# yumingj/C2-Matching

Hardware: AMD Instinct MI355X
Metric: LR-Ref image pairs/sec (160x160 LR, 500x500 Ref, 4x SR) (higher is better)
Workload: dtype f32

## Files before the change

c2-matching_amd/c2m_amd/_lib.py:

```python
import ctypes
import os

import torch

_HERE = os.path.dirname(os.path.abspath(__file__))
LIB_PATH = os.environ.get("C2M_LIB") or os.path.join(os.path.dirname(_HERE), "csrc", "libc2m_hip.so")
ABI_VERSION = 5

_vp, _i, _sz = ctypes.c_void_p, ctypes.c_int, ctypes.c_size_t
_lib = None


class ConvSrc(ctypes.Structure):
    _fields_ = [("ptr", _vp), ("C", _i), ("pix_pitch", _i), ("row_pitch", _i), ("img_pitch", ctypes.c_longlong)]


class Conv3x3Desc(ctypes.Structure):
    _fields_ = [("B", _i), ("H", _i), ("W", _i), ("Cin", _i), ("Cout", _i), ("nsrc", _i), ("src", ConvSrc * 2),
                ("wr", _vp), ("bias", _vp), ("act", _i), ("slope", ctypes.c_float), ("out_mode", _i), ("out", _vp),
                ("out_pix_pitch", _i), ("out_row_pitch", _i), ("out_img_pitch", ctypes.c_longlong), ("res1", _vp),
                ("res2", _vp), ("mask_out", _vp), ("flow", _vp), ("fh", _i), ("fw", _i), ("scale", _i), ("n_off", _i),
                ("abs_sum", _vp), ("algo", _i), ("cout_offset", _i), ("cout_total", _i),
                ("out2", _vp), ("out2_row_pitch", _i), ("out2_plane_pitch", ctypes.c_longlong),
                ("out2_img_pitch", ctypes.c_longlong), ("range_flag", _vp), ("io_flags", ctypes.c_int)]


class ImageSrc(ctypes.Structure):
    _fields_ = [("ptr", _vp), ("pix_pitch", ctypes.c_longlong), ("row_pitch", ctypes.c_longlong),
                ("plane_pitch", ctypes.c_longlong), ("img_pitch", ctypes.c_longlong)]


class C2MError(RuntimeError):
    pass


def _declare(L):
    L.c2m_abi_version.restype = _i
    L.c2m_status_string.restype = ctypes.c_char_p
    L.c2m_status_string.argtypes = [_i]
    L.c2m_last_hip_error.restype = ctypes.c_char_p
    L.c2m_device_arch.argtypes = [ctypes.c_char_p, _i]
    L.c2m_profile_enable.argtypes = [_i]
    L.c2m_profile_collect.argtypes = [ctypes.POINTER(ctypes.c_float), ctypes.POINTER(_i), _i, ctypes.POINTER(_i)]
    L.c2m_feature_normalize_f32.argtypes = [_vp, _vp, _i, _i, _i, _vp]
    L.c2m_feature_match_workspace_bytes.restype = _sz
    L.c2m_feature_match_workspace_bytes.argtypes = [_i] * 5
    L.c2m_feature_match_workspace_bytes_c.restype = _sz
    L.c2m_feature_match_workspace_bytes_c.argtypes = [_i] * 6
    L.c2m_feature_match_skip_table.argtypes = [_i] * 5 + [ctypes.POINTER(ctypes.c_size_t), ctypes.POINTER(ctypes.c_int)]
    L.c2m_feature_match_index_f32.argtypes = [_vp, _vp, _vp] + [_i] * 12 + [_vp, _vp, _vp, _sz]
    L.c2m_feature_match_index_pre_f32.argtypes = [_vp, _vp, _vp] + [_i] * 12 + [_vp, _vp, _vp, _sz, _vp, _vp]
    L.c2m_feature_match_index_pre_f32.restype = _i
    L.c2m_feature_normalize_ss_f32.argtypes = [_vp, _vp, _i, _i, _i, _vp, _vp]
    L.c2m_feature_normalize_ss_f32.restype = _i
    L.c2m_feature_match_filter_tables.argtypes = [_i] * 5 + [ctypes.POINTER(ctypes.c_size_t)] * 3 + [ctypes.POINTER(ctypes.c_int)]
    L.c2m_build_pre_offsets_f32.argtypes = [_vp, _vp, _i, _i, _i, _vp, _vp, _vp]
    for name in ("c2m_dcn_v2_forward_workspace_bytes",):
        getattr(L, name).restype = _sz
        getattr(L, name).argtypes = [_i] * 8
    L.c2m_dcn_v2_backward_workspace_bytes.restype = _sz
    L.c2m_dcn_v2_backward_workspace_bytes.argtypes = [_i] * 14
    L.c2m_dcn_v2_forward_f32.argtypes = [_vp] * 6 + [_i] * 14 + [_vp, _vp, _sz]
    L.c2m_dcn_v2_forward_bf16mma_f32.argtypes = [_vp] * 6 + [_i] * 14 + [_vp, _vp, _sz]
    L.c2m_dcn_v2_backward_f32.argtypes = [_vp] * 7 + [_i] * 14 + [_vp] * 5 + [_vp, _sz]
    L.c2m_dcn_fuse_offsets_f32.argtypes = [_vp, _vp, _vp, _i, _i, _i, _i, _i, _vp, _vp, _vp]
    L.c2m_nchw_to_nhwc_bordered_f32.argtypes = [_vp, _vp, _i, _i, _i, _i, _vp]
    L.c2m_dcn_v2_relayout_bytes.restype = _sz
    L.c2m_dcn_v2_relayout_bytes.argtypes = [_i] * 5
    L.c2m_dcn_v2_relayout_f32.argtypes = [_vp, _vp, _i, _i, _i, _i, _i, _vp]
    L.c2m_conv3x3_rgb64_f32.argtypes = [_vp, _vp, _i, _i, _i, _vp, _vp, _vp, _vp, _i, ctypes.c_float, _vp, _i, _i,
                                        ctypes.c_longlong, _vp, _i, ctypes.c_longlong, ctypes.c_longlong]
    L.c2m_dcn_v2_forward_nhwc_f32.argtypes = [_vp] * 6 + [_i] * 14 + [_vp, _i, _i, _i, ctypes.c_longlong, _i, ctypes.c_float, _i]
    L.c2m_dcn_v2_relayout_f16x2_bytes.restype = _sz
    L.c2m_dcn_v2_relayout_f16x2_bytes.argtypes = [_i] * 5
    L.c2m_dcn_v2_relayout_f16x2.argtypes = [_vp, _vp, _i, _i, _i, _i, _i, _vp]
    L.c2m_dcn_v2_forward_nhwc_f16x2.argtypes = [_vp] * 6 + [_i] * 14 + [_vp, _i, _i, _i, ctypes.c_longlong, _i, ctypes.c_float, _i, _vp]
    L.c2m_conv3x3_relayout_bytes.restype = _sz
    L.c2m_conv3x3_relayout_bytes.argtypes = [_i, _i]
    L.c2m_conv3x3_relayout_f32.argtypes = [_vp, _vp, _i, _i, _vp]
    L.c2m_conv3x3_relayout_wino_bytes.restype = _sz
    L.c2m_conv3x3_relayout_wino_bytes.argtypes = [_i, _i]
    L.c2m_conv3x3_relayout_wino_f32.argtypes = [_vp, _vp, _i, _i, _vp]
    L.c2m_conv3x3_relayout_wino4_bytes.restype = _sz
    L.c2m_conv3x3_relayout_wino4_bytes.argtypes = [_i, _i]
    L.c2m_conv3x3_relayout_wino4_f32.argtypes = [_vp, _vp, _i, _i, _vp]
    L.c2m_conv3x3_relayout_split_bytes.restype = _sz
    L.c2m_conv3x3_relayout_split_bytes.argtypes = [_i, _i, _i]
    L.c2m_conv3x3_relayout_split_f32.argtypes = [_vp, _vp, _i, _i, _i, _vp]
    L.c2m_conv3x3_relayout_split_dgrad_f32.argtypes = [_vp, _vp, _i, _i, _i, _vp]
    L.c2m_conv3x3_relayout_split_multi.argtypes = [_vp, _vp, _i, ctypes.c_longlong, _i]
    L.c2m_conv3x3_wgrad_workspace_bytes.restype = _sz
    L.c2m_conv3x3_wgrad_workspace_bytes.argtypes = [_i] * 5
    L.c2m_conv3x3_wgrad_f32.argtypes = [_vp, ctypes.POINTER(ConvSrc), _i, _vp, _i, _i, ctypes.c_longlong] + [_i] * 5 + [_vp, _vp, _sz]
    L.c2m_conv3x3_nhwc_f32.argtypes = [_vp, ctypes.POINTER(Conv3x3Desc)]
    L.c2m_index_to_flow_f32.argtypes = [_vp, _vp, _i, _i, _i, _vp]
    L.c2m_contras_loss_workspace_bytes.restype = _sz
    L.c2m_contras_loss_workspace_bytes.argtypes = [_i] * 6
    L.c2m_contras_loss_forward_f32.argtypes = [_vp] * 5 + [_i] * 6 + [_vp] * 3 + [_i, _i] + [ctypes.c_float] * 3 + [_vp, _vp, _sz]
    L.c2m_contras_loss_rows_f32.argtypes = [_vp] + [_i] * 6 + [_vp, _sz] + [_vp] * 5
    L.c2m_contras_loss_backward_f32.argtypes = [_vp] + [_i] * 6 + [_vp] * 3 + [_i, _i] + [ctypes.c_float] * 3 + [_i] + [_vp] * 4 + [_sz]
    L.c2m_warp_perspective_u8.argtypes = [_vp] * 4 + [_i] * 3 + [_vp] * 3
    L.c2m_pil_bicubic_u8.argtypes = [_vp, _vp] + [_i] * 5 + [_vp] * 3 + [_i, _vp, _vp]
    L.c2m_pil_bicubic2d_lds_bytes.restype = _sz
    L.c2m_pil_bicubic2d_lds_bytes.argtypes = [_i] * 4
    L.c2m_pil_bicubic2d_u8.argtypes = [_vp] * 3 + [_i] * 6 + ([_vp] * 3 + [_i]) * 2 + [_i, _i] + [_vp] * 3
    L.c2m_val_metrics_tile.argtypes = [ctypes.POINTER(_i)] * 2
    L.c2m_val_metrics_workspace_bytes.restype = _sz
    L.c2m_val_metrics_workspace_bytes.argtypes = [_i] * 4
    L.c2m_val_metrics_f32.argtypes = [_vp, ctypes.POINTER(ImageSrc), ctypes.POINTER(ImageSrc)] + [_i] * 7 + [_vp] * 4 + [_sz]


def lib():
    global _lib
    if _lib is None:
        if not os.path.exists(LIB_PATH):
            raise C2MError(f"{LIB_PATH} not found: build it with `python -c 'import __graft_entry__ as g; g.build()'` "
                           "(hipcc --offload-arch=gfx950).  There is no CPU or PyTorch fallback for this path.")
        L = ctypes.CDLL(LIB_PATH)
        _declare(L)
        v = L.c2m_abi_version()
        if v != ABI_VERSION:
            raise C2MError(f"libc2m_hip.so ABI {v} != expected {ABI_VERSION}")
        _lib = L
    return _lib


def check(status, what):
    if status != 0:
        L = lib()
        msg = L.c2m_status_string(status).decode()
        hip = L.c2m_last_hip_error().decode() if status == 4 else ""
        raise C2MError(f"{what}: {msg}" + (f" [{hip}]" if hip else ""))


def device_arch():
    buf = ctypes.create_string_buffer(256)
    check(lib().c2m_device_arch(buf, 256), "c2m_device_arch")
    return buf.value.decode()


KERNEL_NAMES = {1: "corr_argmax_mfma", 2: "corr_argmax_generic", 3: "dcn_v2_forward", 4: "dcn_v2_backward_data",
                5: "dcn_v2_backward_weight", 6: "conv3x3_mfma", 7: "conv3x3_split", 8: "conv3x3_wgrad", 9: "corr_filter",
                10: "corr_resolve"}


def profile_enable(on=True):
    check(lib().c2m_profile_enable(int(bool(on))), "c2m_profile_enable")


def profile_collect(capacity=512):
    ms = (ctypes.c_float * capacity)()
    ids = (_i * capacity)()
    n = _i(0)
    check(lib().c2m_profile_collect(ms, ids, capacity, ctypes.byref(n)), "c2m_profile_collect")
    return [(KERNEL_NAMES.get(ids[k], str(ids[k])), float(ms[k])) for k in range(n.value)]
```

c2-matching_amd/c2m_amd/ops.py:

```python
import collections
import ctypes
import os
import threading
import warnings
import weakref

import torch

from . import _lib


def _dev_f32(t, name):
    if not isinstance(t, torch.Tensor) or not t.is_cuda:
        raise _lib.C2MError(f"{name} must be a tensor on the GPU (the HIP path has no CPU fallback)")
    if t.dtype != torch.float32:
        raise _lib.C2MError(f"{name} must be float32, got {t.dtype}")
    return t if t.is_contiguous() else t.contiguous()


def _stream():
    return torch.cuda.current_stream().cuda_stream


def _pair(v):
# ... 377 lines not shown
                                        "job table would need a host-to-device copy); run one eager forward before capturing")
                rowsl, first = [], 0
                for (wptr, iptr, ci, co, flags, elems) in jobs:
                    rowsl.append([wptr, iptr, ci, co, flags, elems, first, 0])
                    first += (elems + 255) // 256
                host = torch.tensor(rowsl, dtype=torch.int64).pin_memory()
                tab = (sig, host.to(dev, non_blocking=True), first, int(any((j[4] & 0xf) == 2 for j in jobs)), host)
                if len(self._tables) >= 64:
                    self._tables.clear()
                self._tables[tkey] = tab
            with torch.cuda.device(dev):
                _lib.check(_lib.lib().c2m_conv3x3_relayout_split_multi(_stream(), tab[1].data_ptr(), len(jobs), tab[2], tab[3]),
                           "c2m_conv3x3_relayout_split_multi")
        return n

    @staticmethod
    def _relayout(weight, rows, pad_cin_to, kind, wr=None):
        w = weight.detach()
        if rows is not None:
            w = w[rows[0]:rows[1]]
        if w.dtype != torch.float32 or not w.is_cuda or w.dim() != 4 or tuple(w.shape[2:]) != (3, 3):
            raise _lib.C2MError("conv3x3: weight must be a float32 GPU tensor [Cout, Cin, 3, 3]")
        Co, Ci = w.shape[:2]
        if pad_cin_to is not None and Ci < pad_cin_to:
            w = torch.nn.functional.pad(w, (0, 0, 0, 0, 0, pad_cin_to - Ci))
            Ci = pad_cin_to
        w = w.contiguous()
        L, k = _lib.lib(), _KINDS[kind]
        args = ((Co, Ci) if k.swap else (Ci, Co)) + ((k.pieces,) if k.pieces else ())
        nbytes = getattr(L, k.size_fn)(*args)
        if nbytes == 0:
            raise _lib.C2MError(f"conv3x3: unsupported channel counts Cin={Ci}, Cout={Co}" + (" for this kernel" if kind else
                                " (input channels must be a multiple of 32)"))
        if wr is None:
            wr = torch.empty((nbytes + 3) // 4, dtype=torch.float32, device=w.device)
        with torch.cuda.device(w.device):
            _lib.check(getattr(L, k.relayout_fn)(_stream(), w.data_ptr(), Ci, Co, *args[2:], wr.data_ptr()), k.relayout_fn)
        return wr

    def get(self, weight, pad_cin_to=None, rows=None, kind=K_DIRECT):
        key = (weight.data_ptr(), weight._version, tuple(weight.shape), pad_cin_to, weight.device.index)
        slot = (id(weight), rows, kind)
        hit = self._lookup(slot, key, weight)
        if hit is not None:
            return hit
        wr = self._relayout(weight, rows, pad_cin_to, kind)
        self._store(slot, key, weight, wr,
                    redo=lambda w, buf, rows=rows, pad=pad_cin_to, kind=kind: self._relayout(w, rows, pad, kind, buf))
        return wr


_wcache = _WeightCache()


def _nhwc_src(t, name, bf16_ok=False):
    if not t.is_cuda or t.dim() != 4 or not (t.dtype == torch.float32 or (bf16_ok and t.dtype == torch.bfloat16)):
        raise _lib.C2MError(f"{name} must be a 4-D float32 GPU tensor" + (" (or bfloat16)" if bf16_ok else ""))
    sb, sc, sh, sw = t.stride()
    if sc != 1:
        raise _lib.C2MError(f"{name} must be channels-last (stride 1 along C); got strides {t.stride()}")
    B, C, H, W = t.shape
    if W == 1 and sw % 8 != 0:
        sw = (C + 7) // 8 * 8
    if H == 1 and sh % 8 != 0:
        sh = W * sw
    if B == 1 and sb % 8 != 0:
        sb = H * sh
    return _lib.ConvSrc(t.data_ptr(), C, sw, sh, sb)


def empty_nhwc(B, C, H, W, device, dtype=torch.float32):
    return torch.empty((B, C, H, W), dtype=dtype, device=device, memory_format=torch.channels_last)


_SPLIT = os.environ.get("C2M_CONV_SPLIT", "all")
_SPLIT16 = os.environ.get("C2M_CONV_SPLIT16", "1") != "0"


def experimental_built():
    return False


_DCN_F16X2 = os.environ.get("C2M_DCN_F16X2", "1") != "0"


_tls = threading.local()
_range_flags = {}
_range_lock = threading.Lock()


def _device_flag(dev):
    key = (dev.type, dev.index if dev.index is not None else torch.cuda.current_device())
    t = _range_flags.get(key)
    if t is None:
        with _range_lock:
            t = _range_flags.get(key)
            if t is None:
                t = _range_flags[key] = torch.zeros(1, dtype=torch.int32, device=dev)
    return t


def _range_flag(dev):
    g = getattr(_tls, "guard_flag", None)
    if g is not None and g.device == (dev if dev.index is not None else torch.device(dev.type, torch.cuda.current_device())):
        return g
    return _device_flag(dev)


def _f16x2_auto():
    ov = getattr(_tls, "flavour", None)
    if ov is not None:
        return ov
    if getattr(_tls, "guarded", False):
        return _SPLIT16
    if _SPLIT16 and not _f16x2_auto.warned and not torch.cuda.is_current_stream_capturing():
        _f16x2_auto.warned = True
        warnings.warn("c2m_amd.ops: a conv3x3 / conv3x3_dcn_head / dcn_v2_forward_nhwc call outside `f16_range_guard` and without "
                      "`ops.conv_flavour(...)` runs the FULL-RANGE arithmetic (bf16 x 3 convolutions, fp32-MFMA DCNv2: ~2x the matrix "
                      "work of the f16 x 2 default of the fused module forwards).  For f16 x 2 wrap the calls in "
                      "`with ops.conv_flavour('f16x2'):` and poll `ops.range_flag_set(device)` (domain |x| < 65520); "
                      "`with ops.conv_flavour('bf16x3'):` silences this.", RuntimeWarning, stacklevel=3)
    return False


_f16x2_auto.warned = False


def range_flag_set(device, clear=True):
    f = _device_flag(torch.device("cuda", device) if isinstance(device, int) else torch.device(device))
    v = int(f.item()) != 0
    if clear and v:
        f.zero_()
    return v


class conv_flavour:

    def __init__(self, name):
        if name not in ("f16x2", "bf16x3"):
            raise _lib.C2MError("conv_flavour: 'f16x2' or 'bf16x3'")
        self.val = name == "f16x2"

    def __enter__(self):
        self.prev = getattr(_tls, "flavour", None)
        _tls.flavour = self.val
        return self

    def __exit__(self, *exc):
        _tls.flavour = self.prev
        return False


def f16_range_guard(owner, fn, device):
    if getattr(_tls, "guarded", False):
        return fn()
    if getattr(owner, "_c2m_conv_bf16x3", False):
        with conv_flavour("bf16x3"):
            return fn()
    ov = getattr(_tls, "flavour", None)
    if not (_SPLIT16 if ov is None else ov):
        return fn()
    if torch.cuda.is_current_stream_capturing():
        with conv_flavour("bf16x3"):
            return fn()
    flag = torch.zeros(1, dtype=torch.int32, device=device)
    _tls.guarded, _tls.guard_flag = True, flag
    try:
        out = fn()
    finally:
        _tls.guarded, _tls.guard_flag = False, None
    if int(flag.item()) == 0:
        return out
    warnings.warn(f"{type(owner).__name__}: an activation left the f16 x 2 convolution flavour's domain (|x| >= 65520); the forward "
                  "was recomputed on the bf16 x 3 flavour (full fp32 range), which this module now keeps", RuntimeWarning)
    try:
        owner._c2m_conv_bf16x3 = True
    except Exception:
        pass
    with conv_flavour("bf16x3"):
        return fn()


def _wino_ok(srcs, weight, out_mode, W):
    return (out_mode in ("nhwc", "nhwc_pool2") and weight.shape[0] % 64 == 0 and W % 32 == 0 and
            all(s.shape[1] % 16 == 0 for s in srcs) and sum(s.shape[1] for s in srcs) == weight.shape[1])


def _wino4_ok(srcs, weight, out_mode, W):
    return W % 64 == 0 and out_mode == "nhwc" and _wino_ok(srcs, weight, out_mode, W)


def bf16_autocast():
    return torch.is_autocast_enabled('cuda') and torch.get_autocast_dtype('cuda') == torch.bfloat16


def _split_ok(srcs, weight, fast):
    return ((_SPLIT == "all" or (fast and _SPLIT != "0")) and all(s.shape[1] % 16 == 0 for s in srcs) and
            sum(s.shape[1] for s in srcs) == weight.shape[1])


def _as_list(srcs):
    return list(srcs) if isinstance(srcs, (list, tuple)) else [srcs]


def _check_abs_sum(abs_sum):
    if abs_sum is not None and (abs_sum.dtype != torch.float64 or abs_sum.numel() < 256 or not abs_sum.is_cuda):
        raise _lib.C2MError("abs_sum must be a float64 GPU tensor with 256 slots (C2M_ABS_SUM_SLOTS)")


def _split_kind(algo):
    if algo == "bf16" or (algo is None and bf16_autocast()):
        return K_BF16
    if algo == "split16" or (algo is None and _f16x2_auto()):
        return K_SPLIT16
    return K_SPLIT


def _conv_desc(kind, srcs, wr, B, H, W, Cin, Cout, names=None, bf16_ok=False):
    d = _lib.Conv3x3Desc()
    d.algo = _KINDS[kind].algo
    d.B, d.H, d.W, d.Cin, d.Cout, d.nsrc = B, H, W, Cin, Cout, len(srcs)
    for k, s in enumerate(srcs):
        if tuple(s.shape[2:]) != (H, W) or s.shape[0] != B:
            raise _lib.C2MError("conv3x3: sources must share B, H, W")
        d.src[k] = _nhwc_src(s, names[k] if names else f"src{k}", bf16_ok=bf16_ok)
    d.wr = wr.data_ptr()
    if kind == K_SPLIT16:
        d.range_flag = _range_flag(srcs[0].device).data_ptr()
    return d


def _desc_out(d, out, bf16_ok=False):
    o = _nhwc_src(out, "out", bf16_ok=bf16_ok)
    d.out, d.out_pix_pitch, d.out_row_pitch, d.out_img_pitch = out.data_ptr(), o.pix_pitch, o.row_pitch, o.img_pitch
    return o


def _launch_conv(d, dev, kind, family_prefix=""):
    with torch.cuda.device(dev):
        _lib.check(_lib.lib().c2m_conv3x3_nhwc_f32(_stream(), d), "c2m_conv3x3_nhwc_f32")
    if _ConvFlops.enabled:
        f = 2.0 * d.Cout * 9 * d.Cin * d.H * d.W * d.B
        _ConvFlops.add(family_prefix + _KINDS[kind].family, f, f * _KINDS[kind].exec_factor)


def conv3x3(srcs, weight, bias=None, act=ACT_NONE, slope=0.1, res1=None, res2=None, out_mode="nhwc", out=None, algo=None,
            out2_grouped8=None, fast=False, out_dtype=None, dword_stores=False):
    srcs = _as_list(srcs)
    B, _, H, W = srcs[0].shape
    Cin = sum(s.shape[1] for s in srcs)
    Cout = weight.shape[0]
    dev = srcs[0].device
    if algo is None:
        reduced = bf16_autocast()
        if (out2_grouped8 is None and (_split_ok(srcs, weight, fast) or (reduced and _split_ok(srcs, weight, True))) and (out_mode != "nhwc_pool2" or (H % 2 == 0 and W % 2 == 0))
                and (out_mode not in ("nhwc", "nhwc_pool2") or Cout % 4 == 0)):
            kind = _split_kind(None)
        else:
            kind = K_WINO4 if (fast and _wino4_ok(srcs, weight, out_mode, W)) else K_WINO if _wino_ok(srcs, weight, out_mode, W) else K_DIRECT
    elif algo in ALGO_IDS:
        kind = ALGO_IDS[algo]
    else:
        raise _lib.C2MError(f"conv3x3: unknown algo {algo!r} (one of {', '.join(ALGO_IDS)})")
    if out2_grouped8 is not None:
        if algo not in (None, "direct") or out_mode != "nhwc":
            raise _lib.C2MError("out2_grouped8 needs the direct kernel in nhwc mode")
        kind = K_DIRECT
    wr = _wcache.get(weight, pad_cin_to=Cin if weight.shape[1] < Cin else None, kind=kind)
    d = _conv_desc(kind, srcs, wr, B, H, W, Cin, Cout, bf16_ok=True)
    io = 1 if srcs[0].dtype == torch.bfloat16 else 0
    if any(s.dtype == torch.bfloat16 for s in srcs[1:]) or (io and len(srcs) != 1):
        raise _lib.C2MError("conv3x3: a bfloat16 source must be the only source")
    if out is not None:
        out_dtype = out.dtype
    if out_dtype == torch.bfloat16:
        io |= 2
    elif out_dtype not in (None, torch.float32):
        raise _lib.C2MError("conv3x3: out_dtype is float32 or bfloat16")
    for bit, r in ((4, res1), (8, res2)):
        if r is not None and r.dtype == torch.bfloat16:
            io |= bit
    if io and (kind != K_BF16 or out_mode != "nhwc"):
        raise _lib.C2MError("conv3x3: bfloat16 tensors need the bf16 kernel (algo='bf16' / bf16 autocast) in nhwc mode")
    if dword_stores:
        if io or kind not in _SPLIT_KINDS or out_mode not in ("pixel_shuffle", "nchw"):
            raise _lib.C2MError("conv3x3: dword_stores selects a store path of the split kernels' pixel_shuffle / nchw epilogues")
        io = 16
    d.io_flags = io
    if bias is not None:
        bias = _dev_f32(bias.detach(), "bias")
    d.bias = bias.data_ptr() if bias is not None else None
    d.act, d.slope = int(act), float(slope)
    if out_mode == "nhwc":
        if out is None:
            out = empty_nhwc(B, Cout, H, W, dev, torch.bfloat16 if io & 2 else torch.float32)
        d.out_mode = 0
        o = _desc_out(d, out, bf16_ok=True)
        for name, r in (("res1", res1), ("res2", res2)):
            if r is not None:
                rs = _nhwc_src(r, name, bf16_ok=True)
                if (rs.pix_pitch, rs.row_pitch, rs.img_pitch) != (o.pix_pitch, o.row_pitch, o.img_pitch) or r.shape != out.shape:
                    raise _lib.C2MError(f"{name} must have the geometry of the output")
                setattr(d, name, r.data_ptr())
        if out2_grouped8 is not None:
            d.out2, d.out2_row_pitch, d.out2_plane_pitch, d.out2_img_pitch = _grouped8_args(out2_grouped8, B, Cout, H, W, dev)
    elif out_mode == "pixel_shuffle":
        out = empty_nhwc(B, Cout // 4, 2 * H, 2 * W, dev)
        d.out_mode = 1
        _desc_out(d, out)
    elif out_mode == "nhwc_pool2":
        if kind not in _POOL_KINDS or H % 2 != 0 or W % 2 != 0:
            raise _lib.C2MError("conv3x3: the pooled epilogue needs the Winograd F(2,3) or the split-bf16 kernel and even H, W")
        out = empty_nhwc(B, Cout, H // 2, W // 2, dev)
        d.out_mode = 4
        _desc_out(d, out)
    elif out_mode == "nchw":
        out = torch.empty((B, Cout, H, W), dtype=torch.float32, device=dev)
        d.out_mode = 2
        d.out = out.data_ptr()
    else:
        raise _lib.C2MError(f"unknown out_mode {out_mode}")
    _launch_conv(d, dev, kind)
    return out


def conv3x3_dgrad(grad_out, weight):
    Cout, Cin = weight.shape[:2]
    B, Cg, H, W = grad_out.shape
    if Cg != Cout or Cout % 16 != 0 or Cin % 4 != 0:
        raise _lib.C2MError("conv3x3_dgrad: grad_out channels must equal weight.shape[0] (a multiple of 16); Cin % 4 == 0")
    wr = _wcache.get(weight, kind=K_DGRAD)
    out = empty_nhwc(B, Cin, H, W, grad_out.device)
    d = _conv_desc(K_DGRAD, [grad_out], wr, B, H, W, Cout, Cin, names=("grad_out",))
    d.out_mode = 0
    _desc_out(d, out)
    _launch_conv(d, grad_out.device, K_DGRAD)
    return out


def conv3x3_wgrad(srcs, grad_out, Cout):
    srcs = _as_list(srcs)
    B, _, H, W = srcs[0].shape
    Cin = sum(s_.shape[1] for s_ in srcs)
    if tuple(grad_out.shape) != (B, Cout, H, W):
        raise _lib.C2MError("conv3x3_wgrad: grad_out must be [B, Cout, H, W]")
    dev = grad_out.device
    L = _lib.lib()
    arr = (_lib.ConvSrc * 2)()
    for k, s_ in enumerate(srcs):
        arr[k] = _nhwc_src(s_, f"src{k}")
    g = _nhwc_src(grad_out, "grad_out")
    gw = torch.empty((Cout, Cin, 3, 3), dtype=torch.float32, device=dev)
    with torch.cuda.device(dev):
        nbytes = L.c2m_conv3x3_wgrad_workspace_bytes(B, H, W, Cin, Cout)
        ws = torch.empty(max(nbytes, 4) // 4, dtype=torch.float32, device=dev)
        _lib.check(L.c2m_conv3x3_wgrad_f32(_stream(), arr, len(srcs), grad_out.data_ptr(), g.pix_pitch, g.row_pitch, g.img_pitch,
                                           B, H, W, Cin, Cout, gw.data_ptr(), ws.data_ptr(), nbytes), "c2m_conv3x3_wgrad_f32")
    return gw


def _as_nhwc(t):
    t = t.float() if t.dtype != torch.float32 else t
    return t if t.stride(1) == 1 else t.contiguous(memory_format=torch.channels_last)


class _Conv3x3Fn(torch.autograd.Function):

    @staticmethod
    def forward(ctx, weight, bias, act, slope, *srcs):
        srcs = [_as_nhwc(s_) for s_ in srcs]
        out = conv3x3(srcs, weight, bias, act=act, slope=slope, algo="split")
        ctx.act, ctx.slope, ctx.nsrc = int(act), float(slope), len(srcs)
        ctx.save_for_backward(weight, *(srcs + ([out] if act != ACT_NONE else [])))
        return out

    @staticmethod
    @torch.autograd.function.once_differentiable
    def backward(ctx, grad_out):
        saved = ctx.saved_tensors
        weight, srcs = saved[0], list(saved[1:1 + ctx.nsrc])
        g = _as_nhwc(grad_out)
        if ctx.act != ACT_NONE:
            out = saved[1 + ctx.nsrc]
            g = g * torch.where(out > 0, 1.0, ctx.slope if ctx.act == ACT_LRELU else 0.0)
            g = _as_nhwc(g)
        need = ctx.needs_input_grad
        gw = conv3x3_wgrad(srcs, g, weight.shape[0]) if need[0] else None
        gb = g.sum(dim=(0, 2, 3)) if need[1] else None
        gsrc = [None] * ctx.nsrc
        if any(need[4:4 + ctx.nsrc]):
            Co = weight.shape[0]
            if Co % 16 != 0:
                pad = 16 - Co % 16
                dx = conv3x3_dgrad(_as_nhwc(torch.nn.functional.pad(g, (0, 0, 0, 0, 0, pad))),
                                   torch.nn.functional.pad(weight.detach(), (0, 0, 0, 0, 0, 0, 0, pad)))
            else:
                dx = conv3x3_dgrad(g, weight)
            c0 = 0
            for k, s_ in enumerate(srcs):
                if need[4 + k]:
                    gsrc[k] = dx[:, c0:c0 + s_.shape[1]]
                c0 += s_.shape[1]
        return (gw, gb, None, None, *gsrc)


def conv3x3_autograd(srcs, weight, bias=None, act=ACT_NONE, slope=0.1):
    srcs = _as_list(srcs)
    return _Conv3x3Fn.apply(weight, bias, int(act), float(slope), *srcs)


def conv3x3_autograd_ok(srcs, weight):
    srcs = _as_list(srcs)
    return (all(s_.is_cuda and s_.dim() == 4 and s_.shape[1] % 32 == 0 for s_ in srcs) and weight.shape[0] % 4 == 0 and
            sum(s_.shape[1] for s_ in srcs) == weight.shape[1] and tuple(weight.shape[2:]) == (3, 3) and _SPLIT != "0")


def _grouped8_args(g2, B, Cout, H, W, dev):
    if g2 is None:
        return None, 0, 0, 0
    if (g2.dtype != torch.float32 or not g2.is_contiguous() or Cout % 8 != 0 or
            tuple(g2.shape) != (B, Cout // 8, H + 3, W + 3, 8) or g2.device != dev):
        raise _lib.C2MError("out2_grouped8 must be a contiguous float32 [B, Cout/8, H+3, W+3, 8] buffer")
    return g2.data_ptr() + ((W + 3) + 1) * 8 * 4, (W + 3) * 8, (H + 3) * (W + 3) * 8, (Cout // 8) * (H + 3) * (W + 3) * 8


def conv3x3_rgb64(image, weight, bias=None, act=ACT_NONE, slope=0.1, mean=None, std=None, out=None, out2_grouped8=None):
    if image.dim() != 4 or image.shape[1] != 3 or not image.is_cuda:
        raise _lib.C2MError("conv3x3_rgb64: image must be a GPU tensor [B,3,H,W]")
    if tuple(weight.shape) != (64, 3, 3, 3):
        raise _lib.C2MError("conv3x3_rgb64: weight must be [64,3,3,3]")
    B, _, H, W = image.shape
    if (mean is None) != (std is None):
        raise _lib.C2MError("conv3x3_rgb64: mean and std go together")
    if 12 * H * W >= 2 ** 31:
        raise _lib.C2MError(f"conv3x3_rgb64: image of {H} x {W} pixels is too large (H * W < 178 956 971)")
    x = image.float().contiguous()
    dev = x.device
    w = _dev_f32(weight.detach(), "weight")
    bias = _dev_f32(bias.detach(), "bias") if bias is not None else None
    if mean is not None:
        mean, std = _dev_f32(mean.detach().reshape(3), "mean"), _dev_f32(std.detach().reshape(3), "std")
    if out is None:
        out = empty_nhwc(B, 64, H, W, dev)
    o = _nhwc_src(out, "out")
    if tuple(out.shape) != (B, 64, H, W):
        raise _lib.C2MError("conv3x3_rgb64: out must be [B,64,H,W]")
    o2, o2_row, o2_plane, o2_img = _grouped8_args(out2_grouped8, B, 64, H, W, dev)
    with torch.cuda.device(dev):
        _lib.check(_lib.lib().c2m_conv3x3_rgb64_f32(
            _stream(), x.data_ptr(), B, H, W, w.data_ptr(), bias.data_ptr() if bias is not None else None,
            mean.data_ptr() if mean is not None else None, std.data_ptr() if std is not None else None, int(act),
            float(slope), out.data_ptr(), o.pix_pitch, o.row_pitch, o.img_pitch, o2, o2_row, o2_plane, o2_img),
            "c2m_conv3x3_rgb64_f32")
    if _ConvFlops.enabled:
        _ConvFlops.add("rgb_first_layer", 2.0 * 64 * 27 * H * W * B, 2.0 * 64 * 28 * H * W * B)
    return out


def index_to_flow(max_idx):
    if not max_idx.is_cuda or max_idx.dtype != torch.int64 or max_idx.dim() != 3:
        raise _lib.C2MError("max_idx must be an int64 GPU tensor [B, hq, wq]")
    mi = max_idx.contiguous()
    B, hq, wq = mi.shape
    flow = torch.empty((B, hq, wq, 2), dtype=torch.float32, device=mi.device)
    with torch.cuda.device(mi.device):
        _lib.check(_lib.lib().c2m_index_to_flow_f32(_stream(), mi.data_ptr(), B, hq, wq, flow.data_ptr()), "c2m_index_to_flow_f32")
    return flow


def conv3x3_dcn_head(srcs, weight, bias, deformable_groups, flow=None, scale=1, abs_sum=None, algo=None, dword_stores=False):
    srcs = _as_list(srcs)
    B, _, H, W = srcs[0].shape
    Cin = sum(s.shape[1] for s in srcs)
    dg = int(deformable_groups)
    Cout = weight.shape[0]
    if Cout != 3 * dg * 9:
        raise _lib.C2MError("conv3x3_dcn_head: weight must have 3*dg*9 output channels")
    dev = srcs[0].device
    bias = _dev_f32(bias.detach(), "bias")
    offset = torch.empty((B, 2 * dg * 9, H, W), dtype=torch.float32, device=dev)
    mask = torch.empty((B, dg * 9, H, W), dtype=torch.float32, device=dev)
    if flow is not None:
        if flow.dtype != torch.float32 or not flow.is_cuda or flow.dim() != 4 or flow.shape[0] != B or flow.shape[3] != 2:
            raise _lib.C2MError("flow must be float32 [B, fh, fw, 2] on the GPU")
        flow = flow.contiguous()
    _check_abs_sum(abs_sum)
    split = (Cout // 64) * 64
    slices = [(0, Cout)] if (split == 0 or Cout - split > 32 or split == Cout) else [(0, split), (split, Cout)]
    use_split = algo in ("split", "bf16", "split16") or (algo is None and _SPLIT != "0" and all(s_.shape[1] % 16 == 0 for s_ in srcs))
    split_kind = _split_kind(algo)
    wino = algo is None and W % 32 == 0 and all(s_.shape[1] % 16 == 0 for s_ in srcs)
    if dword_stores and not use_split:
        raise _lib.C2MError("conv3x3_dcn_head: dword_stores selects a store path of the split kernels' epilogue")
    for (c0, c1) in slices:
        kind = split_kind if use_split else K_WINO if (wino and (c1 - c0) % 64 == 0) else K_DIRECT
        wr = _wcache.get(weight, rows=(c0, c1), kind=kind)
        d = _conv_desc(kind, srcs, wr, B, H, W, Cin, c1 - c0)
        d.bias = bias.data_ptr() + 4 * c0
        d.out_mode = 3
        d.out, d.mask_out, d.n_off, d.scale = offset.data_ptr(), mask.data_ptr(), 2 * dg * 9, int(scale)
        d.cout_offset, d.cout_total = c0, Cout
        if flow is not None:
            d.flow, d.fh, d.fw = flow.data_ptr(), flow.shape[1], flow.shape[2]
        if abs_sum is not None:
            d.abs_sum = abs_sum.data_ptr()
        if dword_stores:
            d.io_flags = 16
        _launch_conv(d, dev, kind, "dcn_head_")
    return offset, mask


class BorderedNHWC:
    grouped8 = None

    def __new__(cls, x=None):
        pre = bordered_of(x) if x is not None else None
        return pre if pre is not None else super().__new__(cls)

    def __init__(self, x):
        if bordered_of(x) is self:
            return
        x = _dev_f32(x, "x")
        self.B, self.C, self.H, self.W = x.shape
        self.buf = torch.empty((self.B, self.H + 3, self.W + 3, self.C), dtype=torch.float32, device=x.device)
        with torch.cuda.device(x.device):
            _lib.check(_lib.lib().c2m_nchw_to_nhwc_bordered_f32(_stream(), x.data_ptr(), self.B, self.C, self.H, self.W,
                                                               self.buf.data_ptr()), "c2m_nchw_to_nhwc_bordered_f32")

    def interior(self):
        return self.buf[:, 1:self.H + 1, 1:self.W + 1, :].permute(0, 3, 1, 2)


class _DcnWeightCache(_WeightCache):
    _IMAGES = {K_DCN: ("c2m_dcn_v2_relayout_bytes", "c2m_dcn_v2_relayout_f32", "geometry is not on the channels-last path"),
               K_DCN16: ("c2m_dcn_v2_relayout_f16x2_bytes", "c2m_dcn_v2_relayout_f16x2",
                         "geometry has no f16 x 2 kernel (needs >= 16 channels per (virtual) group)")}

    @classmethod
    def _relayout_dcn(cls, weight, dg, kind, wt=None):
        size_fn, relayout_fn, why = cls._IMAGES[kind]
        w = _dev_f32(weight.detach(), "weight")
        Co, C, kh, kw = w.shape
        L = _lib.lib()
        nbytes = getattr(L, size_fn)(C, Co, kh, kw, dg)
        if nbytes == 0:
            raise _lib.C2MError("dcn_v2_forward_nhwc: " + why)
        if wt is None:
            wt = torch.empty(nbytes // 4, dtype=torch.float32, device=w.device)
        with torch.cuda.device(w.device):
            _lib.check(getattr(L, relayout_fn)(_stream(), w.data_ptr(), C, Co, kh, kw, dg, wt.data_ptr()), relayout_fn)
        return wt

    def get(self, weight, dg, f16x2=False):
        key = (weight.data_ptr(), weight._version, tuple(weight.shape), dg, weight.device.index)
        kind = K_DCN16 if f16x2 else K_DCN
        slot = (id(weight), None, kind)
        hit = self._lookup(slot, key, weight)
        if hit is not None:
            return hit
        wt = self._relayout_dcn(weight, dg, kind)
        self._store(slot, key, weight, wt, redo=lambda w, buf, dg=dg, kind=kind: self._relayout_dcn(w, dg, kind, buf))
        return wt


_dcn_wcache = _DcnWeightCache()


def refresh_weight_caches(module_or_params=None, all_kinds=False):
    ids = None
    if module_or_params is not None:
        params = module_or_params.parameters() if hasattr(module_or_params, "parameters") else module_or_params
        ids = {id(p) for p in params}
    kinds = None
    if not all_kinds and not torch.is_grad_enabled():
        kinds = {*_MFMA32_KINDS, _split_kind(None)}
    return _wcache.refresh(ids, kinds) + _dcn_wcache.refresh(ids)


def clear_weight_caches():
    _wcache.clear()
    _dcn_wcache.clear()


def dcn_f16x2_ok(weight, deformable_groups):
    Co, C, kh, kw = weight.shape
    return _lib.lib().c2m_dcn_v2_relayout_f16x2_bytes(C, Co, kh, kw, int(deformable_groups)) != 0


def dcn_v2_forward_nhwc(inp_bordered, weight, bias, offset, mask, deformable_groups, act=ACT_NONE, slope=0.1,
                        nhwc_out=True, algo=None):
    if not isinstance(inp_bordered, BorderedNHWC):
        raise _lib.C2MError("inp_bordered must be a BorderedNHWC")
    B, C, H, W = inp_bordered.B, inp_bordered.C, inp_bordered.H, inp_bordered.W
    Co = weight.shape[0]
    dg = int(deformable_groups)
    offset, mask, bias = _dev_f32(offset, "offset"), _dev_f32(mask, "mask"), _dev_f32(bias.detach(), "bias")
    _check_offset_mask(offset, mask, B, dg, 9, H, W, ("9", "H", "W"))
    if algo is None:
        f16 = _DCN_F16X2 and _SPLIT != "0" and _f16x2_auto() and dcn_f16x2_ok(weight, dg)
    elif algo in ("fp32", "f16x2"):
        f16 = algo == "f16x2"
    else:
        raise _lib.C2MError("dcn_v2_forward_nhwc: algo is None, 'fp32' or 'f16x2'")
    wt = _dcn_wcache.get(weight, dg, f16x2=f16)
    dev = offset.device
    if nhwc_out:
        out = empty_nhwc(B, Co, H, W, dev)
        o = _nhwc_src(out, "out")
        pitches = (1, o.pix_pitch, o.row_pitch, o.img_pitch)
    else:
        out = torch.empty((B, Co, H, W), dtype=torch.float32, device=dev)
        pitches = (0, 0, 0, 0)
    grouped = inp_bordered.grouped8 is not None and C == 8 * dg
    src = inp_bordered.grouped8 if grouped else inp_bordered.buf
    fn = "c2m_dcn_v2_forward_nhwc_f16x2" if f16 else "c2m_dcn_v2_forward_nhwc_f32"
    with torch.cuda.device(dev):
        tail = (_range_flag(dev).data_ptr(),) if f16 else ()
        _lib.check(getattr(_lib.lib(), fn)(_stream(), src.data_ptr(), wt.data_ptr(), bias.data_ptr(), offset.data_ptr(),
                                           mask.data_ptr(), B, C, H, W, Co, 3, 3, 1, 1, 1, 1, 1, 1, dg, out.data_ptr(), *pitches,
                                           int(act), float(slope), int(grouped), *tail), fn)
    return out


def _bordered_empty(B, C, H, W, device, grouped8=False):
    def zero_border(t):
        t[..., 0, :, :].zero_()
        t[..., H + 1:, :, :].zero_()
        t[..., 1:H + 1, 0, :].zero_()
        t[..., 1:H + 1, W + 1:, :].zero_()
        return t

    o = BorderedNHWC.__new__(BorderedNHWC)
    o.B, o.C, o.H, o.W = B, C, H, W
    o.buf = zero_border(torch.empty((B, H + 3, W + 3, C), dtype=torch.float32, device=device))
    if grouped8:
        if C % 8 != 0:
            raise _lib.C2MError("a group-major twin needs C % 8 == 0")
        o.grouped8 = zero_border(torch.empty((B, C // 8, H + 3, W + 3, 8), dtype=torch.float32, device=device))
    return o


def bordered_of(t):
    return getattr(t, "_c2m_bordered", None)


def _pool_is_2x2(m):
    two = lambda v: v in (2, (2, 2))
    return two(m.kernel_size) and two(m.stride) and m.padding in (0, (0, 0)) and m.dilation in (1, (1, 1)) and not m.ceil_mode


def vgg_stack_forward(layers, x, taps=(), mean=None, std=None, last_nchw=False, grouped8_taps=(), fast=False):
    names = list(layers.keys())
    B, C, H, W = x.shape
    dev = x.device
    refresh_weight_caches([p_ for layer_ in layers.values() for p_ in layer_.parameters()])
    first = layers[names[0]]
    rgb64 = C == 3 and isinstance(first, torch.nn.Conv2d) and tuple(first.weight.shape) == (64, 3, 3, 3)
    if rgb64:
        cur = x
    else:
        cur = torch.zeros((B, 32, H, W), dtype=torch.float32, device=dev).contiguous(memory_format=torch.channels_last)
        xin = x.float()
        if mean is not None:
            xin = (xin - mean) / std
        cur[:, :C] = xin
    out, k = {}, 0

    def conv(k_, src, layer_, **kw):
        if k_ == 0 and rgb64:
            kw.pop("algo", None)
            return conv3x3_rgb64(src, layer_.weight, layer_.bias, mean=mean, std=std, **kw)
        return conv3x3(src, layer_.weight, layer_.bias, fast=fast, **kw)

    while k < len(names):
        name, layer = names[k], layers[names[k]]
        if isinstance(layer, torch.nn.Conv2d):
            if layer.kernel_size != (3, 3) or layer.stride != (1, 1) or layer.padding != (1, 1) or layer.groups != 1:
                raise _lib.C2MError(f"vgg_stack_forward: {name} is not a 3x3 / stride 1 / pad 1 convolution")
            relu = k + 1 < len(names) and isinstance(layers[names[k + 1]], torch.nn.ReLU)
            tap_name = names[k + 1] if (relu and names[k + 1] in taps) else (name if name in taps and not relu else None)
            if name in taps and relu:
                raise _lib.C2MError("tapping a conv output that is followed by an in-place ReLU is not supported")
            last = (k + (2 if relu else 1)) >= len(names)
            Bc, _, Hc, Wc = cur.shape
            nxt = layers[names[k + 2]] if (relu and k + 2 < len(names)) else None
            pool = (isinstance(nxt, torch.nn.MaxPool2d) and _pool_is_2x2(nxt) and tap_name is None and not (k == 0 and rgb64) and
                    Hc % 2 == 0 and Wc % 2 == 0 and
                    (_wino_ok([cur], layer.weight, "nhwc_pool2", Wc) or _split_ok([cur], layer.weight, fast)))
            if last and last_nchw:
                cur = conv3x3(cur, layer.weight, layer.bias, act=ACT_RELU if relu else ACT_NONE, out_mode="nchw", fast=fast)
                out[names[k + 1] if relu else name] = cur
            elif tap_name is not None:
                bo = _bordered_empty(Bc, layer.out_channels, Hc, Wc, dev, grouped8=tap_name in grouped8_taps)
                view = bo.interior()
                conv(k, cur, layer, act=ACT_RELU if relu else ACT_NONE, out=view, out2_grouped8=bo.grouped8)
                view._c2m_bordered = bo
                out[tap_name] = view
                cur = view
            elif pool:
                cur = conv3x3(cur, layer.weight, layer.bias, act=ACT_RELU, out_mode="nhwc_pool2", fast=fast)
                k += 1
            else:
                cur = conv(k, cur, layer, act=ACT_RELU if relu else ACT_NONE)
            k += 2 if relu else 1
        elif isinstance(layer, torch.nn.MaxPool2d):
            cur = torch.nn.functional.max_pool2d(cur, layer.kernel_size, layer.stride, layer.padding)
            k += 1
        elif isinstance(layer, torch.nn.ReLU):
            cur = torch.relu(cur)
            k += 1
        else:
            raise _lib.C2MError(f"vgg_stack_forward: unsupported layer {name}: {type(layer).__name__}")
    return out



CONTRAS_MIN_IDS = 128


def contras_correspondences(transformed_coordinates, H1, W1, scaling_steps=2, min_ids=CONTRAS_MIN_IDS):
    tc = transformed_coordinates[:, ::4, ::4, :2]
    B = tc.shape[0]
    if tc.shape[1] != H1 or tc.shape[2] != W1:
        raise ValueError(f"transformed_coordinates[:, ::4, ::4] is {tuple(tc.shape[1:3])}, the feature grid is {(H1, W1)}")
    x = tc[..., 0].reshape(B, -1)
    y = tc[..., 1].reshape(B, -1)
    valid = (x > 10) & (x < 4 * W1 - 10) & (y > 10) & (y < 4 * H1 - 10)
    keep = valid.sum(1) >= min_ids
    valid = valid & keep[:, None]
    counts = valid.sum(1)
    nz = valid.nonzero()
    bi, ids = nz[:, 0], nz[:, 1]
    div = float(2 ** scaling_steps)
    pos2 = torch.stack([torch.round(y[bi, ids] / div), torch.round(x[bi, ids] / div)], 1).to(torch.int32)
    offsets = torch.zeros(B + 1, dtype=torch.int32, device=tc.device)
    offsets[1:] = torch.cumsum(counts, 0).to(torch.int32)
    return {"ids": ids.to(torch.int32).contiguous(), "pos2": pos2.contiguous(), "offsets": offsets, "keep": keep,
            "counts": [int(c) for c in counts.cpu()], "n_valid": int(keep.sum())}


class _ContrasLossFn(torch.autograd.Function):

    @staticmethod
    def forward(ctx, f1, f2, tf1, tf2, corr, margin, safe_radius, temperature):
        B, C, H1, W1 = f1.shape
        H2, W2 = f2.shape[2], f2.shape[3]
        teacher = tf1 is not None
        Ntot, max_n = int(corr["ids"].numel()), max(corr["counts"])
        L = _lib.lib()
        nbytes = L.c2m_contras_loss_workspace_bytes(B, C, H1, W1, Ntot, int(teacher))
        if nbytes == 0:
            raise _lib.C2MError("c2m_contras_loss_workspace_bytes: invalid shapes")
        ws = torch.empty(nbytes, dtype=torch.uint8, device=f1.device)
        out = torch.empty((B, 4), dtype=torch.float32, device=f1.device)
        with torch.cuda.device(f1.device):
            _lib.check(L.c2m_contras_loss_forward_f32(
                _stream(), f1.data_ptr(), f2.data_ptr(), tf1.data_ptr() if teacher else None,
                tf2.data_ptr() if teacher else None, B, C, H1, W1, H2, W2, corr["ids"].data_ptr(), corr["pos2"].data_ptr(),
                corr["offsets"].data_ptr(), Ntot, max_n, float(margin), float(safe_radius), float(temperature),
                out.data_ptr(), ws.data_ptr(), nbytes), "c2m_contras_loss_forward_f32")
        ctx.meta = (B, C, H1, W1, H2, W2, Ntot, max_n, float(margin), float(safe_radius), float(temperature), teacher, nbytes)
        ctx.corr = corr
        corr["_workspace"] = ws
        ctx.save_for_backward(ws)
        dists = out[:, 1:3].contiguous()
        ctx.mark_non_differentiable(dists)
        return out[:, 0::3].contiguous(), dists

    @staticmethod
    def backward(ctx, g_terms, g_dists):
        (ws,) = ctx.saved_tensors
        B, C, H1, W1, H2, W2, Ntot, max_n, margin, radius, tau, teacher, nbytes = ctx.meta
        corr = ctx.corr
        g_terms = (g_terms if g_terms is not None else torch.zeros((B, 2), device=ws.device)).float().contiguous()
        gf1 = torch.empty((B, C, H1, W1), dtype=torch.float32, device=ws.device)
        gf2 = torch.empty((B, C, H2, W2), dtype=torch.float32, device=ws.device)
        with torch.cuda.device(ws.device):
            _lib.check(_lib.lib().c2m_contras_loss_backward_f32(
                _stream(), B, C, H1, W1, H2, W2, corr["ids"].data_ptr(), corr["pos2"].data_ptr(),
                corr["offsets"].data_ptr(), Ntot, max_n, margin, radius, tau, int(teacher), g_terms.data_ptr(),
                gf1.data_ptr(), gf2.data_ptr(), ws.data_ptr(), nbytes), "c2m_contras_loss_backward_f32")
        return gf1, gf2, None, None, None, None, None, None


def contras_loss(f1, f2, transformed_coordinates, margin=1.0, safe_radius=4, scaling_steps=2, teacher=None,
                 temperature=0.15, distill_weight=15.0):
    f1, f2 = _dev_f32(f1, "f1"), _dev_f32(f2, "f2")
    if f1.dim() != 4 or f2.dim() != 4 or f1.shape[:2] != f2.shape[:2] or f1.device != f2.device:
        raise _lib.C2MError("f1 / f2 must be [B,C,H,W] with equal B, C and device")
    tf1 = tf2 = None
    if teacher is not None:
        tf1, tf2 = (_dev_f32(t.detach(), n) for t, n in zip(teacher, ("teacher f1", "teacher f2")))
        if tf1.shape != f1.shape or tf2.shape != f2.shape:
            raise _lib.C2MError("teacher features must have the student's shapes")
    if not isinstance(transformed_coordinates, torch.Tensor) or not transformed_coordinates.is_cuda:
        raise _lib.C2MError("transformed_coordinates must be a tensor on the GPU")
    B, C, H1, W1 = f1.shape
    corr = contras_correspondences(transformed_coordinates.to(f1.device), H1, W1, scaling_steps)
    if corr["n_valid"] == 0:
        raise NotImplementedError("no sample has 128 valid correspondences")
    H2, W2 = f2.shape[2], f2.shape[3]
    if corr["pos2"].numel():
        lim = torch.stack([corr["pos2"].min(0).values, corr["pos2"].max(0).values]).cpu()
        if int(lim[0].min()) < 0 or int(lim[1, 0]) >= H2 or int(lim[1, 1]) >= W2:
            raise IndexError(f"pos2 outside the {H2}x{W2} map of f2")
    terms, dists = _ContrasLossFn.apply(f1, f2, tf1, tf2, corr, margin, safe_radius, temperature)
    wgt = corr["keep"].to(torch.float32)
    n = float(corr["n_valid"])
    if teacher is None:
        loss = (terms[:, 0] * wgt).sum().view(1) / n
    else:
        loss = ((terms[:, 0] + distill_weight * terms[:, 1]) * wgt).sum().view(1) / n
    pos_dist = (dists[:, 0] * wgt).sum() / n
    neg_dist = (dists[:, 1] * wgt).sum() / n
    if teacher is None:
        return loss, pos_dist, neg_dist
    return loss, pos_dist, neg_dist, (terms[:, 1] * wgt).sum() / n


def contras_loss_rows(f1, f2, transformed_coordinates, margin=1.0, safe_radius=4, scaling_steps=2, teacher=None,
                      temperature=0.15):
    f1, f2 = _dev_f32(f1, "f1"), _dev_f32(f2, "f2")
    B, C, H1, W1 = f1.shape
    corr = contras_correspondences(transformed_coordinates.to(f1.device), H1, W1, scaling_steps)
    if corr["n_valid"] == 0:
        raise NotImplementedError("no sample has 128 valid correspondences")
    tf1, tf2 = (None, None) if teacher is None else (_dev_f32(teacher[0], "teacher f1"), _dev_f32(teacher[1], "teacher f2"))
    with torch.no_grad():
        _ContrasLossFn.apply(f1, f2, tf1, tf2, corr, margin, safe_radius, temperature)
    ws = corr.pop("_workspace")
    N = int(corr["ids"].numel())
    rows = {k: torch.empty(N, dtype=torch.float32, device=f1.device) for k in ("pos", "neg1", "neg2")}
    rows.update({k: torch.empty(N, dtype=torch.int32, device=f1.device) for k in ("neg1_idx", "neg2_idx")})
    with torch.cuda.device(f1.device):
        _lib.check(_lib.lib().c2m_contras_loss_rows_f32(
            _stream(), B, C, H1, W1, N, int(teacher is not None), ws.data_ptr(), ws.numel(), rows["pos"].data_ptr(),
            rows["neg1"].data_ptr(), rows["neg1_idx"].data_ptr(), rows["neg2"].data_ptr(), rows["neg2_idx"].data_ptr()),
            "c2m_contras_loss_rows_f32")
    rows.update(corr)
    return rows



_PIL_PRECISION_BITS = 32 - 8 - 2


def _dev_u8(t, name):
    if not isinstance(t, torch.Tensor) or not t.is_cuda:
        raise _lib.C2MError(f"{name} must be a tensor on the GPU (the HIP path has no CPU fallback)")
    if t.dtype != torch.uint8:
        raise _lib.C2MError(f"{name} must be uint8, got {t.dtype}")
    return t if t.is_contiguous() else t.contiguous()


def _pil_bicubic_weight(x):
    a = -0.5
    x = abs(x)
    if x < 1.0:
        return ((a + 2.0) * x - (a + 3.0)) * x * x + 1
    if x < 2.0:
        return (((x - 5) * x + 8) * x - 4) * a
    return 0.0
# ... 290 lines not shown
```

c2-matching_amd/csrc/conv3x3.hip:

```cpp
#include <stdio.h>
#include <stdlib.h>

#include <type_traits>

#include "c2m_common.h"
#include "conv3x3_shared.h"

namespace c2m {
namespace conv {

constexpr int TW = 32, TH = 4;
constexpr int HW_ = TW + 2, HH_ = TH + 2;
constexpr int NPIX = HW_ * HH_;
constexpr int KCH = 32;
constexpr int NIN_REAL = (NPIX * 8 + 63) / 64;
constexpr int NIN_W = 7;
constexpr int IN_BYTES = NIN_REAL * 1024;
static_assert(NIN_REAL <= 4 * NIN_W, "four waves x NIN_W instructions must cover the halo tile");

__global__ void __launch_bounds__(256) conv3x3_relayout_kernel(const float* __restrict__ w, int Cin, int Cout, int MW,
                                                                 long long total, float* __restrict__ wr) {
  const long long e0 = (long long)blockIdx.x * 256 + threadIdx.x;
  if (e0 >= total + 64) return;
  if (e0 >= total) { wr[e0] = 0.0f; return; }
// ... 1046 lines not shown
  const int wv = __builtin_amdgcn_readfirstlane(tid >> 6);

  float wreg[14][2];
#pragma unroll
  for (int t = 0; t < 14; ++t) {
    int c, dy, dx;
    bool live = true;
    if (t < 9) { c = t / 3; dy = t % 3; dx = hi; }
    else if (t < 12) { c = t - 9; dy = hi; dx = 2; }
    else if (t == 12) { c = hi; dy = 2; dx = 2; }
    else { c = 2; dy = 2; dx = 2; live = hi == 0; }
#pragma unroll
    for (int mt = 0; mt < 2; ++mt) wreg[t][mt] = live ? p.w[(size_t)(mt * 32 + j) * 27 + c * 9 + dy * 3 + dx] : 0.0f;
  }
  const unsigned lds0 = (unsigned)(uintptr_t)(__attribute__((address_space(3))) float*)&tile[0][0];
  const unsigned pix = (unsigned)(j * 4);
  const unsigned bA = pix + hi * 4;
  const unsigned bB = pix + hi * (CHW * 4) + 8;
  const unsigned bC = pix + hi * (PLANE * 4) + (2 * CHW + 2) * 4;
  const unsigned bD = pix + (2 * PLANE + 2 * CHW + 2) * 4;

  int s_off[EPT], s_ry[EPT], s_rx[EPT], s_c[EPT];
#pragma unroll
  for (int i = 0; i < EPT; ++i) {
    const int e = tid + 256 * i;
    const int c = e / PLANE, rem = e - c * PLANE;
    s_c[i] = e < NEL ? c : -1;
    s_ry[i] = rem / CHW;
    s_rx[i] = rem - s_ry[i] * CHW;
    s_off[i] = e;
  }
  float mean_[3] = {0.0f, 0.0f, 0.0f}, std3[3] = {1.0f, 1.0f, 1.0f};
  if (p.mean) {
#pragma unroll
    for (int c = 0; c < 3; ++c) { mean_[c] = p.mean[c]; std3[c] = p.std_[c]; }
  }
  const int ntile = p.tiles_x * p.tiles_y * p.B;
  float stage[EPT];
  unsigned okm = 0u;
  const unsigned in_bytes = (unsigned)(3 * p.H * p.W) * 4u;
  auto fetch = [&](int t) __attribute__((always_inline)) {
    const int tx = t % p.tiles_x, ty = (t / p.tiles_x) % p.tiles_y, b = t / (p.tiles_x * p.tiles_y);
    const __amdgpu_buffer_rsrc_t irs =
        __builtin_amdgcn_make_buffer_rsrc(const_cast<float*>(p.in + (size_t)b * 3 * p.H * p.W), 0, (int)in_bytes, 0x00020000);
    okm = 0u;
#pragma unroll
    for (int i = 0; i < EPT; ++i) {
      const int y = ty * CTH - 1 + s_ry[i], x = tx * CTW - 1 + s_rx[i];
      const unsigned bad = (s_c[i] < 0) | (y < 0) | (y >= p.H) | (x < 0) | (x >= p.W);
      const unsigned off = (unsigned)((s_c[i] * p.H + y) * p.W + x) * 4u;
      stage[i] = __builtin_bit_cast(float, __builtin_amdgcn_raw_buffer_load_b32(irs, off | (bad << 31), 0, 0));
      okm |= (bad ^ 1u) << i;
    }
  };
  auto staged = [&](int i) __attribute__((always_inline)) {
    const int c_lo = (256 * i) / PLANE, c_hi = (256 * i + 255) / PLANE > 2 ? 2 : (256 * i + 255) / PLANE;
    const bool up = c_hi != c_lo && tid + 256 * i >= c_hi * PLANE;
    const float m = up ? mean_[c_hi] : mean_[c_lo], sd = up ? std3[c_hi] : std3[c_lo];
    const float v = (stage[i] - m) / sd;
    return ((okm >> i) & 1u) ? v : 0.0f;
  };
  float bias4[2][4][4];
#pragma unroll
  for (int mt = 0; mt < 2; ++mt)
#pragma unroll
    for (int qd = 0; qd < 4; ++qd)
#pragma unroll
      for (int e = 0; e < 4; ++e) bias4[mt][qd][e] = p.bias ? p.bias[mt * 32 + 8 * qd + 4 * hi + e] : 0.0f;

#pragma unroll
  for (int k = 0; k < 14; ++k) asm volatile("" ::"v"(wreg[k][0]), "v"(wreg[k][1]));
#pragma unroll
  for (int mt = 0; mt < 2; ++mt)
#pragma unroll
    for (int qd = 0; qd < 4; ++qd) asm volatile("" ::"v"(bias4[mt][qd][0]), "v"(bias4[mt][qd][1]), "v"(bias4[mt][qd][2]), "v"(bias4[mt][qd][3]));
  asm volatile("" ::"v"(mean_[0]), "v"(mean_[1]), "v"(mean_[2]), "v"(std3[0]), "v"(std3[1]), "v"(std3[2]));
  auto stage_to = [&](float* buf) __attribute__((always_inline)) {
#pragma unroll
    for (int i = 0; i < EPT; ++i)
      if (256 * (i + 1) <= NEL || s_c[i] >= 0) buf[s_off[i]] = staged(i);
  };
  int t = blockIdx.x;
  if (t < ntile) {
    fetch(t);
    stage_to(tile[0]);
  }
  for (int it = 0; t < ntile; t += gridDim.x, ++it) {
    __syncthreads();
    fetch(min(t + (int)gridDim.x, ntile - 1));
    const int tx = t % p.tiles_x, ty = (t / p.tiles_x) % p.tiles_y, b = t / (p.tiles_x * p.tiles_y);
    const unsigned tb = lds0 + (it & 1) * (NEL * 4);
    float* const obase = p.out + (size_t)b * p.out_img_pitch + (size_t)(ty * CTH) * p.out_row_pitch;
    const __amdgpu_buffer_rsrc_t ors = __builtin_amdgcn_make_buffer_rsrc(obase, 0, (int)p.out_bytes, 0x00020000);
    float* const obase2 = OUT2 ? p.out2 + (size_t)b * p.out2_img_pitch + (size_t)(ty * CTH) * p.out2_row_pitch : obase;
#pragma unroll
    for (int g = 0; g < 4; ++g) {
      const int row = 2 * wv + (g >> 1), col = 32 * (g & 1);
      const unsigned gb = tb + (row * CHW + col) * 4;
      float bv[14];
#pragma unroll
      for (int k = 0; k < 9; ++k)
        bv[k] = *(const __attribute__((address_space(3))) float*)(gb + bA + ((k / 3) * PLANE + (k % 3) * CHW) * 4);
#pragma unroll
      for (int k = 0; k < 3; ++k) bv[9 + k] = *(const __attribute__((address_space(3))) float*)(gb + bB + k * PLANE * 4);
      bv[12] = *(const __attribute__((address_space(3))) float*)(gb + bC);
      bv[13] = *(const __attribute__((address_space(3))) float*)(gb + bD);
      f32x16 acc[2];
#pragma unroll
      for (int mt = 0; mt < 2; ++mt)
#pragma unroll
        for (int r = 0; r < 16; ++r) acc[mt][r] = 0.0f;
#pragma unroll
      for (int k = 0; k < 14; ++k)
#pragma unroll
        for (int mt = 0; mt < 2; ++mt) acc[mt] = __builtin_amdgcn_mfma_f32_32x32x2f32(wreg[k][mt], bv[k], acc[mt], 0, 0, 0);
      const int y = ty * CTH + row, x = tx * CTW + col + j;
      {
        const unsigned bad = (unsigned)(y >= p.H) | (unsigned)(x >= p.W);
        const unsigned ob = ((unsigned)(row * p.out_row_pitch + x * p.out_pix_pitch + 4 * hi) * 4u) | (bad << 31);
        const unsigned ob2 = ((unsigned)(row * p.out2_row_pitch + x * 8 + 4 * hi) * 4u) | (bad << 31);
#pragma unroll
        for (int mt = 0; mt < 2; ++mt)
#pragma unroll
          for (int qd = 0; qd < 4; ++qd) {
            f32x4 v;
#pragma unroll
            for (int e = 0; e < 4; ++e) {
              v[e] = acc[mt][4 * qd + e] + bias4[mt][qd][e];
              if (ACT == 1) v[e] = fmaxf(v[e], 0.0f);
              else if (ACT == 2) v[e] = fmaxf(v[e], v[e] * p.slope);
            }
            __builtin_amdgcn_raw_buffer_store_b128(__builtin_bit_cast(u32x4_t, v), ors, ob + (unsigned)((mt * 32 + 8 * qd) * 4), 0, 0);
            if (OUT2) {
              const __amdgpu_buffer_rsrc_t ors2 = __builtin_amdgcn_make_buffer_rsrc(
                  obase2 + (size_t)(mt * 4 + qd) * p.out2_plane_pitch, 0, (int)p.out2_bytes, 0x00020000);
              __builtin_amdgcn_raw_buffer_store_b128(__builtin_bit_cast(u32x4_t, v), ors2, ob2, 0, 0);
            }
          }
      }
    }
    stage_to(tile[(it + 1) & 1]);
  }
}

}
}

using namespace c2m;

namespace c2m {
namespace conv {
size_t split_relayout_bytes(int Cin, int Cout, int np);
int split_relayout(hipStream_t st, const float* weight, int Cin, int Cout, int np, void* wr, int dgrad);
int launch_split(hipStream_t st, Params p, int np);
int split_relayout_multi(hipStream_t st, const long long* jobs, int njobs, long long nblocks, int any_f16);
}
}

extern "C" size_t c2m_conv3x3_relayout_split_bytes(int Cin, int Cout, int pieces) { return conv::split_relayout_bytes(Cin, Cout, pieces); }

extern "C" int c2m_conv3x3_relayout_split_f32(c2m_stream_t stream, const float* weight, int Cin, int Cout, int pieces, void* wr) {
  if (!weight || !wr) return C2M_ERR_INVALID_ARG;
  return conv::split_relayout(as_stream(stream), weight, Cin, Cout, pieces, wr, 0);
}

extern "C" int c2m_conv3x3_relayout_split_multi(c2m_stream_t stream, const long long* jobs, int njobs, long long nblocks, int any_f16) {
  return conv::split_relayout_multi(as_stream(stream), jobs, njobs, nblocks, any_f16);
}

extern "C" int c2m_conv3x3_relayout_split_dgrad_f32(c2m_stream_t stream, const float* weight, int Cin, int Cout, int pieces, void* wr) {
  if (!weight || !wr) return C2M_ERR_INVALID_ARG;
  return conv::split_relayout(as_stream(stream), weight, Cout, Cin, pieces, wr, 1);
}

namespace {
inline int conv_mw(int Cout) { return 32 * conv::cout_tiles(Cout); }
inline long long relayout_elems(int Cin, int Cout) {
  const int MW = conv_mw(Cout), ncb = (Cout + MW - 1) / MW;
  return (long long)ncb * (Cin / conv::KCH) * 9 * MW * 32;
}
}

extern "C" size_t c2m_conv3x3_relayout_bytes(int Cin, int Cout) {
  if (Cin <= 0 || Cout <= 0 || Cin % conv::KCH != 0) return 0;
  return (size_t)(relayout_elems(Cin, Cout) + 64) * sizeof(float);
}

extern "C" int c2m_conv3x3_relayout_f32(c2m_stream_t stream, const float* weight, int Cin, int Cout, float* wr) {
  if (!weight || !wr || Cin <= 0 || Cout <= 0) return C2M_ERR_INVALID_ARG;
  if (Cin % conv::KCH != 0) return C2M_ERR_UNSUPPORTED;
  const long long total = relayout_elems(Cin, Cout);
  hipLaunchKernelGGL(conv::conv3x3_relayout_kernel, dim3((unsigned)((total + 64 + 255) / 256)), dim3(256), 0,
                     as_stream(stream), weight, Cin, Cout, conv_mw(Cout), total, wr);
  return check_launch();
}

extern "C" size_t c2m_conv3x3_relayout_wino4_bytes(int Cin, int Cout) {
  if (Cin <= 0 || Cout <= 0 || Cin % conv::wino4::KC != 0 || Cout % 64 != 0) return 0;
  return (size_t)(Cout / 64) * (Cin / conv::wino4::KC) * 18 * conv::wino4::WIMG;
}

extern "C" int c2m_conv3x3_relayout_wino4_f32(c2m_stream_t stream, const float* weight, int Cin, int Cout, float* wr) {
  if (!weight || !wr) return C2M_ERR_INVALID_ARG;
  const size_t bytes = c2m_conv3x3_relayout_wino4_bytes(Cin, Cout);
  if (bytes == 0) return C2M_ERR_UNSUPPORTED;
  const long long total = (long long)(bytes / 4);
  hipLaunchKernelGGL(conv::conv3x3_relayout_wino4_kernel, dim3((unsigned)((total + 255) / 256)), dim3(256), 0, as_stream(stream),
                     weight, Cin, Cout, total, wr);
  return check_launch();
}

extern "C" size_t c2m_conv3x3_relayout_wino_bytes(int Cin, int Cout) {
  if (Cin <= 0 || Cout <= 0 || Cin % conv::wino::KC != 0 || Cout % 64 != 0) return 0;
  return (size_t)(Cout / 64) * (Cin / conv::wino::KC) * 12 * conv::wino::WIMG;
}

extern "C" int c2m_conv3x3_relayout_wino_f32(c2m_stream_t stream, const float* weight, int Cin, int Cout, float* wr) {
  if (!weight || !wr) return C2M_ERR_INVALID_ARG;
  const size_t bytes = c2m_conv3x3_relayout_wino_bytes(Cin, Cout);
  if (bytes == 0) return C2M_ERR_UNSUPPORTED;
  const long long total = (long long)(bytes / 4);
  hipLaunchKernelGGL(conv::conv3x3_relayout_wino_kernel, dim3((unsigned)((total + 255) / 256)), dim3(256), 0, as_stream(stream),
                     weight, Cin, Cout, total, wr);
  return check_launch();
}

extern "C" int c2m_conv3x3_rgb64_f32(c2m_stream_t stream, const float* image, int B, int H, int W, const float* weight,
                                     const float* bias, const float* mean, const float* std_, int act, float slope, float* out,
                                     int out_pix_pitch, int out_row_pitch, long long out_img_pitch, float* out2,
                                     int out2_row_pitch, long long out2_plane_pitch, long long out2_img_pitch) {
  if (!image || !weight || !out || B <= 0 || H <= 0 || W <= 0 || (mean == nullptr) != (std_ == nullptr)) return C2M_ERR_INVALID_ARG;
  if (act < 0 || act > 2 || (act == C2M_ACT_LEAKY_RELU && !(slope >= 0.0f && slope <= 1.0f))) return C2M_ERR_UNSUPPORTED;
  if (out_pix_pitch % 4 != 0 || out_row_pitch % 4 != 0 || out_img_pitch % 4 != 0 || ((uintptr_t)out & 15)) return C2M_ERR_UNSUPPORTED;
  if (out2 && (out2_row_pitch % 4 != 0 || out2_plane_pitch % 4 != 0 || out2_img_pitch % 4 != 0 || ((uintptr_t)out2 & 15)))
    return C2M_ERR_UNSUPPORTED;
  conv::c3::Params p;
  p.in = image; p.w = weight; p.bias = bias; p.mean = mean; p.std_ = std_;
  p.B = B; p.H = H; p.W = W;
  p.tiles_x = ceil_div(W, conv::c3::CTW); p.tiles_y = ceil_div(H, conv::c3::CTH);
  p.act = act; p.slope = slope; p.out = out; p.out_pix_pitch = out_pix_pitch; p.out_row_pitch = out_row_pitch;
  p.out_img_pitch = out_img_pitch; p.out2 = out2; p.out2_row_pitch = out2_row_pitch; p.out2_plane_pitch = out2_plane_pitch;
  p.out2_img_pitch = out2_img_pitch;
  const long long ntile = (long long)p.tiles_x * p.tiles_y * B;
  if (ntile > 0x7fffffffLL) return C2M_ERR_INVALID_ARG;
  const long long in_b = 12LL * H * W,
                  out_b = 4LL * ((long long)(conv::c3::CTH - 1) * out_row_pitch + (long long)(W - 1) * out_pix_pitch + 64),
                  out2_b = out2 ? 4LL * ((long long)(conv::c3::CTH - 1) * out2_row_pitch + 8LL * W) : 0;
  if (in_b >= (1LL << 31) || out_b >= (1LL << 31) || out2_b >= (1LL << 31) || out_row_pitch < 0 || out_pix_pitch < 0) return C2M_ERR_UNSUPPORTED;
  p.out_bytes = (unsigned)out_b; p.out2_bytes = (unsigned)out2_b;
  hipStream_t st = as_stream(stream);
  ProfileScope prof(C2M_KERNEL_CONV3X3, st);
  void (*kern)(conv::c3::Params) =
      out2 ? (act == 0 ? &conv::conv3x3_c3_kernel<0, true> : act == 1 ? &conv::conv3x3_c3_kernel<1, true> : &conv::conv3x3_c3_kernel<2, true>)
           : (act == 0 ? &conv::conv3x3_c3_kernel<0, false> : act == 1 ? &conv::conv3x3_c3_kernel<1, false> : &conv::conv3x3_c3_kernel<2, false>);
  hipLaunchKernelGGL(kern, dim3((unsigned)std::min<long long>(ntile, 768)), dim3(256), 0, st, p);
  return check_launch();
}

extern "C" int c2m_index_to_flow_f32(c2m_stream_t stream, const int64_t* max_idx, int B, int hq, int wq, float* flow) {
  if (!max_idx || !flow || B <= 0 || hq <= 0 || wq <= 0) return C2M_ERR_INVALID_ARG;
  const int n = B * hq * wq;
  hipLaunchKernelGGL(conv::index_to_flow_kernel, dim3(ceil_div(n, 256)), dim3(256), 0, as_stream(stream), max_idx, n, hq,
                     wq, reinterpret_cast<float2*>(flow));
  return check_launch();
}

extern "C" int c2m_conv3x3_nhwc_f32(c2m_stream_t stream, const c2m_conv3x3_desc* d) {
  if (!d || !d->wr || !d->out || d->B <= 0 || d->H <= 0 || d->W <= 0 || d->Cin <= 0 || d->Cout <= 0 || d->nsrc < 1 ||
      d->nsrc > 2 || !d->src[0].ptr || (d->nsrc == 2 && !d->src[1].ptr))
    return C2M_ERR_INVALID_ARG;
  const bool wino4 = d->algo == C2M_CONV_WINOGRAD_F43X;
  const bool wino = d->algo == C2M_CONV_WINOGRAD_F23X || wino4;
  const bool splitk = d->algo == C2M_CONV_SPLIT_BF16X3 || d->algo == C2M_CONV_BF16 || d->algo == C2M_CONV_SPLIT_F16X2;
  if (d->algo != 0 && !wino && !splitk) return C2M_ERR_INVALID_ARG;
  if (splitk && (d->out2 || (d->out_mode == 4 && (d->H % 2 != 0 || d->W % 2 != 0 || d->res1 || d->res2)))) return C2M_ERR_UNSUPPORTED;
  if (wino && ((d->out_mode != 0 && d->out_mode != 3 && d->out_mode != 4) || d->Cout % 64 != 0 || d->W % 32 != 0)) return C2M_ERR_UNSUPPORTED;
  if (d->out_mode == 4 && !splitk && (d->algo != C2M_CONV_WINOGRAD_F23X || d->H % 2 != 0 || d->res1 || d->res2 || d->out2)) return C2M_ERR_UNSUPPORTED;
  if (wino4 && (d->out_mode != 0 || d->W % 64 != 0)) return C2M_ERR_UNSUPPORTED;
  const int kch = (wino || splitk) ? conv::wino::KC : conv::KCH;
  int csum = 0;
  for (int s = 0; s < d->nsrc; ++s) {
    if (d->src[s].C <= 0 || d->src[s].C % kch != 0 || d->src[s].pix_pitch % 4 != 0 || d->src[s].row_pitch % 4 != 0 ||
        d->src[s].img_pitch % 4 != 0 || ((uintptr_t)d->src[s].ptr & 15))
      return C2M_ERR_UNSUPPORTED;
    csum += d->src[s].C;
  }
  if (csum != d->Cin || d->H >= 32768 || d->W >= 65536) return C2M_ERR_INVALID_ARG;
  if (d->out_mode < 0 || d->out_mode > 4) return C2M_ERR_INVALID_ARG;
  const bool out_vec4 = !(d->out_pix_pitch % 4 != 0 || d->out_row_pitch % 4 != 0 || d->out_img_pitch % 4 != 0 ||
                          ((uintptr_t)d->out & 15) || ((uintptr_t)d->res1 & 15) || ((uintptr_t)d->res2 & 15));
  if (d->out_mode == 1 && d->Cout % 4 != 0) return C2M_ERR_INVALID_ARG;
  const int cout_total = d->cout_total > 0 ? d->cout_total : d->Cout;
  if (d->out_mode == 3 && (!d->mask_out || d->n_off <= 0 || d->n_off % 4 != 0 || d->n_off >= cout_total || d->scale <= 0 ||
                           d->cout_offset < 0 || d->cout_offset % 4 != 0 || d->cout_offset + d->Cout > cout_total ||
                           (d->flow && (d->fh <= 0 || d->fw <= 0))))
    return C2M_ERR_INVALID_ARG;
  if ((d->res1 || d->res2) && d->out_mode != 0) return C2M_ERR_UNSUPPORTED;

  conv::Params p;
  p.B = d->B; p.H = d->H; p.W = d->W; p.Cin = d->Cin; p.Cout = d->Cout;
  p.tiles_x = ceil_div(d->W, wino4 ? conv::wino4::TWX : wino ? 32 : conv::TW);
  p.tiles_y = ceil_div(d->H, wino4 ? conv::wino4::THY : wino ? 8 : conv::TH);
  p.nchunks = d->Cin / kch;
  for (int s = 0; s < 2; ++s) {
    const int k = s < d->nsrc ? s : 0;
    p.src[s].ptr = d->src[k].ptr; p.src[s].C = s < d->nsrc ? d->src[k].C : 0; p.src[s].pix_pitch = d->src[k].pix_pitch;
    p.src[s].row_pitch = d->src[k].row_pitch; p.src[s].img_pitch = d->src[k].img_pitch;
  }
  p.wr = d->wr; p.wr_zero_off = relayout_elems(d->Cin, d->Cout);
  p.bias = d->bias; p.act = d->act; p.slope = d->slope; p.out_mode = d->out_mode; p.out = d->out;
  p.out_pix_pitch = d->out_pix_pitch; p.out_row_pitch = d->out_row_pitch; p.out_img_pitch = d->out_img_pitch;
  p.res1 = d->res1; p.res2 = d->res2; p.mask_out = d->mask_out; p.flow = d->flow; p.fh = d->fh; p.fw = d->fw;
  p.scale = d->scale; p.n_off = d->n_off; p.abs_sum = d->abs_sum;
  p.scale_shift = -1;
  for (int sh = 0; sh < 16; ++sh)
    if (d->scale == (1 << sh)) p.scale_shift = sh;
  if (d->out_mode == 3 && d->flow && p.scale_shift < 0) return C2M_ERR_UNSUPPORTED;
  if (d->out_mode == 3 && (long long)std::max(d->n_off, cout_total - d->n_off) * d->H * d->W * 4 >= 0x7fffffffLL) return C2M_ERR_UNSUPPORTED;
  p.out_vec4 = out_vec4 ? 1 : 0;
  p.co_off = d->out_mode == 3 ? d->cout_offset : 0;
  p.cout_total = cout_total;
  p.out2 = d->out2; p.out2_row_pitch = d->out2_row_pitch; p.out2_plane_pitch = d->out2_plane_pitch;
  p.out2_img_pitch = d->out2_img_pitch;
  p.range_flag = d->range_flag;
  p.io_flags = d->io_flags;
  if (d->io_flags & C2M_IO_DWORD_STORES) {
    if (!splitk || d->out_mode < 1 || d->out_mode > 3 || (d->io_flags & ~C2M_IO_DWORD_STORES)) return C2M_ERR_UNSUPPORTED;
  } else if (d->io_flags != 0) {
    if (d->algo != C2M_CONV_BF16 || d->out_mode != 0 || (d->io_flags & ~15)) return C2M_ERR_UNSUPPORTED;
    if ((d->io_flags & C2M_IO_SRC_BF16) && (d->nsrc != 1 || d->src[0].pix_pitch % 8 != 0 || d->src[0].row_pitch % 8 != 0 || d->src[0].img_pitch % 8 != 0))
      return C2M_ERR_UNSUPPORTED;
    if (d->Cout % ((d->io_flags & C2M_IO_OUT_BF16) ? 8 : 4) != 0) return C2M_ERR_UNSUPPORTED;
    if ((d->io_flags & C2M_IO_OUT_BF16) && (d->out_pix_pitch % 8 != 0 || d->out_row_pitch % 8 != 0 || d->out_img_pitch % 8 != 0)) return C2M_ERR_UNSUPPORTED;
  }
  if (d->out2 && (wino || d->out_mode != 0 || !out_vec4 || d->Cout % 8 != 0 || ((uintptr_t)d->out2 & 15) ||
                  d->out2_row_pitch % 4 != 0 || d->out2_plane_pitch % 4 != 0 || d->out2_img_pitch % 4 != 0))
    return C2M_ERR_UNSUPPORTED;

  const int MW = wino ? 64 : conv_mw(d->Cout);
  const long long ntile = (long long)p.tiles_x * p.tiles_y * p.B;
  if ((wino || splitk) && (d->out_mode == 0 || d->out_mode == 4) && !out_vec4) return C2M_ERR_UNSUPPORTED;
  if (ntile > 0x7fffffffLL) return C2M_ERR_INVALID_ARG;
  if (d->act == C2M_ACT_LEAKY_RELU && !(d->slope >= 0.0f && d->slope <= 1.0f)) return C2M_ERR_UNSUPPORTED;
  for (int sidx = 0; sidx < d->nsrc; ++sidx) {
    const long long ext = ((long long)(d->H - 1) * d->src[sidx].row_pitch + (long long)(d->W - 1) * d->src[sidx].pix_pitch +
                           d->src[sidx].C) * 4;
    if (ext >= 0x7fffffffLL || d->src[sidx].row_pitch < 0 || d->src[sidx].pix_pitch < 0) return C2M_ERR_UNSUPPORTED;
  }
  if (splitk) {
    ProfileScope prof(C2M_KERNEL_CONV3X3_SPLIT, as_stream(stream));
    return conv::launch_split(as_stream(stream), p, d->algo == C2M_CONV_BF16 ? 1 : (d->algo == C2M_CONV_SPLIT_F16X2 ? 2 : 3));
  }
  const int ncb = ceil_div(d->Cout, MW);
  p.tpw = conv::tiles_per_workgroup(ntile, ncb, wino4 ? 256 : 512, 10);
  dim3 grid((unsigned)((ntile + p.tpw - 1) / p.tpw), ncb);
  hipStream_t st = as_stream(stream);
  ProfileScope prof(C2M_KERNEL_CONV3X3, st);
  const size_t lds = wino4  ? 2 * conv::wino4::IN_BYTES + conv::wino4::NRING * conv::wino4::WUNIT + 1024 + 256
                     : wino ? 2 * conv::wino::IN_BYTES + conv::wino::NRING * conv::wino::WUNIT + 1024 + 256
                            : 2 * conv::IN_BYTES + 3 * (size_t)MW * 128 + 1024 + 256;
  struct Kernel { void (*fn)(conv::Params); unsigned long long lds_done; };
  static Kernel wino4_kernel = {&conv::conv3x3_wino4_kernel, 0};
  static Kernel wino_kernels[3] = {
      {&conv::conv3x3_wino_kernel<16, 0>, 0}, {&conv::conv3x3_wino_kernel<16, 3>, 0}, {&conv::conv3x3_wino_kernel<16, 4>, 0}};
  static Kernel direct_kernels[2][4] = {
      {{&conv::conv3x3_kernel<1, 0>, 0}, {&conv::conv3x3_kernel<1, 1>, 0}, {&conv::conv3x3_kernel<1, 2>, 0}, {&conv::conv3x3_kernel<1, 3>, 0}},
      {{&conv::conv3x3_kernel<2, 0>, 0}, {&conv::conv3x3_kernel<2, 1>, 0}, {&conv::conv3x3_kernel<2, 2>, 0}, {&conv::conv3x3_kernel<2, 3>, 0}}};
  Kernel& k = wino4  ? wino4_kernel
              : wino ? wino_kernels[d->out_mode == 3 ? 1 : d->out_mode == 4 ? 2 : 0]
                     : direct_kernels[MW / 32 - 1][d->out_mode];
  const int rc = ensure_dynamic_lds(reinterpret_cast<const void*>(k.fn), lds, k.lds_done);
  if (rc != C2M_OK) return rc;
  hipLaunchKernelGGL(k.fn, grid, dim3(256), lds, st, p);
  return check_launch();
}
```

c2-matching_amd/csrc/conv3x3_shared.h:

```cpp
#pragma once
#include <stdlib.h>

#include "c2m_common.h"

namespace c2m {
namespace conv {

struct Src {
  const float* ptr;
  int C;
  int pix_pitch;
  int row_pitch;
  long long img_pitch;
};

struct Params {
  int B, H, W, Cin, Cout;
  int tiles_x, tiles_y, nchunks;
  Src src[2];
  const float* wr;
  long long wr_zero_off;
  const float* bias;
  int act;
  float slope;
  int out_mode;
  float* out;
  int out_pix_pitch, out_row_pitch;
  long long out_img_pitch;
  const float* res1;
  const float* res2;
  float* mask_out;
  const float* flow;
  int fh, fw, scale, n_off;
  int scale_shift;
  double* abs_sum;
  int out_vec4;
  int tpw;
  int co_off, cout_total;
  float* out2;
  int out2_row_pitch;
  long long out2_plane_pitch, out2_img_pitch;
  int io_flags;
  int* range_flag;
};

inline int cout_tiles(int Cout) { return Cout <= 32 ? 1 : 2; }

inline int tiles_per_workgroup(long long ntile, int ncb, long long resident, int tmax) {
  static const int env_tpw = [] { const char* e = getenv("C2M_CONV_TPW"); return e ? atoi(e) : 0; }();
  if (env_tpw > 0) return env_tpw;
  long long tpw = 1, best = -1;
  for (long long t = 1; t <= tmax; ++t) {
    const long long wgs = ((ntile + t - 1) / t) * ncb;
    const long long cost = ((wgs + resident - 1) / resident) * t;
    if (best < 0 || cost <= best) { best = cost; tpw = t; }
  }
  return (int)tpw;
}

template <int N>
__device__ __forceinline__ void wait_vmcnt() {
  asm volatile("s_waitcnt vmcnt(%0)" ::"n"(N) : "memory");
}

__device__ __forceinline__ __amdgpu_buffer_rsrc_t make_rsrc(const void* base, unsigned bytes) {
  return __builtin_amdgcn_make_buffer_rsrc(const_cast<void*>(base), 0, (int)bytes, 0x00020000);
}
constexpr unsigned kOOB = 0x80000000u;

struct HeadOut {
  __amdgpu_buffer_rsrc_t off, msk;
};
__device__ __forceinline__ HeadOut head_out(const Params& p, int b) {
  const unsigned HWb = (unsigned)(p.H * p.W) * 4u;
  const int nm = p.cout_total - p.n_off;
  HeadOut h;
  h.off = make_rsrc(p.out + (size_t)b * p.n_off * p.H * p.W, (unsigned)p.n_off * HWb);
  h.msk = make_rsrc(p.mask_out + (size_t)b * nm * p.H * p.W, (unsigned)nm * HWb);
  return h;
}
__device__ __forceinline__ float dcn_head_store(const Params& p, const HeadOut& ho, int b, int y, int x, int col_u, int lane_q,
                                                const f32x4& v) {
  const int HWb = p.H * p.W * 4;
  const int co_u = col_u + p.co_off;
  const int co = co_u + lane_q;
  const int pixb = (y * p.W + x) * 4;
  float asum = 0.0f;
  const int vo = pixb + lane_q * HWb;
  if (co_u < p.n_off) {
#pragma unroll
    for (int h2 = 0; h2 < 2; ++h2) {
      const int gt = (co >> 1) + h2, tap = gt % 9;
      const int ki = (tap * 11) >> 5, kj = tap - 3 * ki;
      float fy = 0.0f, fx = 0.0f;
      if (p.flow) {
        const int ys = y - (ki << p.scale_shift), xs = x - (kj << p.scale_shift);
        const int yy = ys >> p.scale_shift, xx = xs >> p.scale_shift;
        const bool ok = (ys >= 0) & (xs >= 0) & (yy < p.fh) & (xx < p.fw);
        const float2 f = reinterpret_cast<const float2*>(p.flow)[(size_t)b * p.fh * p.fw + (ok ? yy * p.fw + xx : 0)];
        const float sc = ok ? (float)p.scale : 0.0f;
        fx = f.x * sc;
        fy = f.y * sc;
      }
      asum += fabsf(v[2 * h2]) + fabsf(v[2 * h2 + 1]);
      __builtin_amdgcn_raw_buffer_store_b32(__builtin_bit_cast(unsigned, v[2 * h2] + fy), ho.off, vo, (co_u + 2 * h2) * HWb, 0);
      __builtin_amdgcn_raw_buffer_store_b32(__builtin_bit_cast(unsigned, v[2 * h2 + 1] + fx), ho.off, vo,
                                            (co_u + 2 * h2 + 1) * HWb, 0);
    }
  } else {
#pragma unroll
    for (int e = 0; e < 4; ++e)
      if (col_u + lane_q + e < p.Cout)
        __builtin_amdgcn_raw_buffer_store_b32(__builtin_bit_cast(unsigned, __builtin_amdgcn_rcpf(1.0f + __expf(-v[e]))), ho.msk, vo,
                                              (co_u - p.n_off + e) * HWb, 0);
  }
  return asum;
}

template <int CTRL>
__device__ __forceinline__ float quad_dpp(float v) {
  return __builtin_bit_cast(float, __builtin_amdgcn_update_dpp(0, __builtin_bit_cast(int, v), CTRL, 0xf, 0xf, true));
}
__device__ __forceinline__ f32x4 quad_transpose(const f32x4& v, int lane) {
  const bool odd = (lane & 1) != 0, up = (lane & 2) != 0;
  const float r0 = quad_dpp<0xB1>(v[0]), r1 = quad_dpp<0xB1>(v[1]), r2 = quad_dpp<0xB1>(v[2]), r3 = quad_dpp<0xB1>(v[3]);
  const float a0 = odd ? r1 : v[0], a1 = odd ? v[1] : r0, a2 = odd ? r3 : v[2], a3 = odd ? v[3] : r2;
  const float t0 = quad_dpp<0x4E>(a0), t1 = quad_dpp<0x4E>(a1), t2 = quad_dpp<0x4E>(a2), t3 = quad_dpp<0x4E>(a3);
  f32x4 o;
  o[0] = up ? t2 : a0; o[1] = up ? t3 : a1; o[2] = up ? a2 : t0; o[3] = up ? a3 : t1;
  return o;
}
struct HeadFlowWin {
  float fx[2], fy[2];
  int wx_row;
};
__device__ __forceinline__ HeadFlowWin head_flow_window(const Params& p, int b, int y, int x0, int l) {
  HeadFlowWin w;
  w.wx_row = (32 >> p.scale_shift) + 2;
#pragma unroll
  for (int r = 0; r < 2; ++r) {
    w.fx[r] = 0.0f; w.fy[r] = 0.0f;
    if (p.flow != nullptr && (r == 0 || p.scale_shift == 0)) {
      const int e = l + 64 * r;
      const int wy = (e >= w.wx_row ? 1 : 0) + (e >= 2 * w.wx_row ? 1 : 0), wx = e - wy * w.wx_row;
      const int Y = (y >> p.scale_shift) - 2 + wy, X = (x0 >> p.scale_shift) - 2 + wx;
      const bool ok = (e < 3 * w.wx_row) & (Y >= 0) & (X >= 0) & (Y < p.fh) & (X < p.fw);
      const float2 f = reinterpret_cast<const float2*>(p.flow)[(size_t)b * p.fh * p.fw + (ok ? Y * p.fw + X : 0)];
      const float sc = ok ? (float)p.scale : 0.0f;
      w.fx[r] = f.x * sc;
      w.fy[r] = f.y * sc;
    }
  }
  return w;
}
__device__ __forceinline__ float dcn_head_store_quad(const Params& p, const HeadOut& ho, int y, int x, int col_u, int lane_q,
                                                     const f32x4& v, int j, const HeadFlowWin& fw, bool valid) {
  typedef unsigned u32x4_t __attribute__((ext_vector_type(4)));
  const int HWb = p.H * p.W * 4;
  const int co_u = col_u + p.co_off;
  const int co = co_u + lane_q;
  float asum = 0.0f;
  f32x4 w;
  const bool is_off = co_u < p.n_off;
  if (is_off) {
#pragma unroll
    for (int h2 = 0; h2 < 2; ++h2) {
      const int gt = (co >> 1) + h2, tap = gt % 9;
      const int ki = (tap * 11) >> 5, kj = tap - 3 * ki;
      const int e = (2 - ki) * fw.wx_row + (j >> p.scale_shift) + 2 - kj;
      const int src = (e & 63) * 4;
      const float fx0 = __builtin_bit_cast(float, __builtin_amdgcn_ds_bpermute(src, __builtin_bit_cast(int, fw.fx[0])));
      const float fy0 = __builtin_bit_cast(float, __builtin_amdgcn_ds_bpermute(src, __builtin_bit_cast(int, fw.fy[0])));
      float fx = fx0, fy = fy0;
      if (p.scale_shift == 0) {
        const float fx1 = __builtin_bit_cast(float, __builtin_amdgcn_ds_bpermute(src, __builtin_bit_cast(int, fw.fx[1])));
        const float fy1 = __builtin_bit_cast(float, __builtin_amdgcn_ds_bpermute(src, __builtin_bit_cast(int, fw.fy[1])));
        fx = e >= 64 ? fx1 : fx0;
        fy = e >= 64 ? fy1 : fy0;
      }
      asum += valid ? fabsf(v[2 * h2]) + fabsf(v[2 * h2 + 1]) : 0.0f;
      w[2 * h2] = v[2 * h2] + fy;
      w[2 * h2 + 1] = v[2 * h2 + 1] + fx;
    }
  } else {
#pragma unroll
    for (int e = 0; e < 4; ++e) w[e] = __builtin_amdgcn_rcpf(1.0f + __expf(-v[e]));
  }
  const f32x4 t = quad_transpose(w, j);
  const int ch = (is_off ? co : co - p.n_off) + (j & 3);
  const unsigned vo = valid ? (unsigned)(ch * HWb + (y * p.W + (x & ~3)) * 4) : kOOB;
  if (is_off) __builtin_amdgcn_raw_buffer_store_b128(__builtin_bit_cast(u32x4_t, t), ho.off, vo, 0, 0);
  else __builtin_amdgcn_raw_buffer_store_b128(__builtin_bit_cast(u32x4_t, t), ho.msk, vo, 0, 0);
  return asum;
}

__device__ __forceinline__ float dcn_head_store2(const Params& p, const HeadOut& ho, int b, int y, int x, int col_u, int lane_q,
                                                 const f32x4& v0, const f32x4& v1) {
  typedef unsigned u32x2 __attribute__((ext_vector_type(2)));
  const int HWb = p.H * p.W * 4;
  const int co_u = col_u + p.co_off;
// ... 42 lines not shown
```

c2-matching_amd/csrc/conv3x3_split.hip:

```cpp
#include <stdio.h>
#include <stdlib.h>

#include <algorithm>
#include <type_traits>

#include "c2m_common.h"
#include "conv3x3_shared.h"

namespace c2m {
namespace conv {
namespace split {

typedef __bf16 bf16x8 __attribute__((ext_vector_type(8)));
typedef unsigned u32x2 __attribute__((ext_vector_type(2)));

constexpr int KC = 16;
constexpr int TWX = 32, THY = 8;
constexpr int HWc = TWX + 2, HHr = THY + 2;
constexpr int NPIX = HWc * HHr;
constexpr int NRAW_W = (NPIX * 4 + 255) / 256;
constexpr int HALFB = NPIX * 16;
static_assert(HALFB % 128 == 64 && HALFB % 16 == 0, "bank phase of the second k half");

template <int FL> struct Flavour;
template <> struct Flavour<1> {
  static constexpr int NPX = 1, NPW = 1, N = 1; static constexpr bool F16 = false;
  static constexpr int W[1] = {0}; static constexpr int X[1] = {0};
};
template <> struct Flavour<3> {
  static constexpr int NPX = 3, NPW = 3, N = 6; static constexpr bool F16 = false;
  static constexpr int W[6] = {2, 0, 1, 1, 0, 0};
  static constexpr int X[6] = {0, 2, 1, 0, 1, 0};
};
template <> struct Flavour<2> {
  static constexpr int NPX = 2, NPW = 2, N = 3; static constexpr bool F16 = true;
  static constexpr int W[3] = {1, 2, 0};
  static constexpr int X[3] = {0, 1, 0};
};
constexpr float F16_LO_SCALE = 2048.0f;
constexpr int npw_of(int fl) { return fl == 1 ? 1 : fl; }
constexpr int npx_of(int fl) { return fl == 2 ? 2 : fl; }

typedef unsigned u32x4 __attribute__((ext_vector_type(4)));
__device__ __forceinline__ void split3(const f32x4 v, u32x2& p0, u32x2& p1, u32x2& p2) {
  const u32x4 m = {0xffff0000u, 0xffff0000u, 0xffff0000u, 0xffff0000u};
  const u32x4 vb = __builtin_bit_cast(u32x4, v);
  const f32x4 r = v - __builtin_bit_cast(f32x4, vb & m);
  const u32x4 rb = __builtin_bit_cast(u32x4, r);
  const f32x4 t = r - __builtin_bit_cast(f32x4, rb & m);
  const u32x4 tb = __builtin_bit_cast(u32x4, t);
  p0 = u32x2{__builtin_amdgcn_perm(vb[1], vb[0], 0x07060302u), __builtin_amdgcn_perm(vb[3], vb[2], 0x07060302u)};
  p1 = u32x2{__builtin_amdgcn_perm(rb[1], rb[0], 0x07060302u), __builtin_amdgcn_perm(rb[3], rb[2], 0x07060302u)};
  p2 = u32x2{__builtin_amdgcn_perm(tb[1], tb[0], 0x07060302u), __builtin_amdgcn_perm(tb[3], tb[2], 0x07060302u)};
}

typedef _Float16 f16x4 __attribute__((ext_vector_type(4)));
typedef _Float16 f16x8 __attribute__((ext_vector_type(8)));
__device__ __forceinline__ void split2_f16(const f32x4 v, u32x2& p0, u32x2& p1) {
  const f16x4 h0 = __builtin_convertvector(v, f16x4);
  const f32x4 r = (v - __builtin_convertvector(h0, f32x4)) * F16_LO_SCALE;
  const f16x4 h1 = __builtin_convertvector(r, f16x4);
  p0 = __builtin_bit_cast(u32x2, h0);
  p1 = __builtin_bit_cast(u32x2, h1);
}

__device__ __forceinline__ float f16_weight_scale(float wmax) {
  if (!(wmax > 0.0f) || wmax > 3.0e38f) return 1.0f;
  int e;
  (void)frexpf(wmax, &e);
  e = 15 - e;
  e = e < -100 ? -100 : (e > 100 ? 100 : e);
  return ldexpf(1.0f, e);
}
__device__ __forceinline__ unsigned short f16_bits(float v) { return __builtin_bit_cast(unsigned short, (_Float16)v); }
__device__ __forceinline__ unsigned short f16_piece(float w, int pl, float S) {
  const float v = w * S;
  const _Float16 a = (_Float16)v;
  if (pl == 0) return __builtin_bit_cast(unsigned short, a);
  return f16_bits(v - (float)a);
}

__device__ __forceinline__ unsigned short bf16_piece(float w, int pl, bool rne) {
  if (rne) {
    unsigned u = __builtin_bit_cast(unsigned, w);
    if ((u & 0x7f800000u) == 0x7f800000u) return (unsigned short)(u >> 16);
    u += 0x7fffu + ((u >> 16) & 1u);
    return (unsigned short)(u >> 16);
  }
  float x = w;
  for (int k = 0; k < pl; ++k) x = x - __builtin_bit_cast(float, __builtin_bit_cast(unsigned, x) & 0xffff0000u);
  return (unsigned short)(__builtin_bit_cast(unsigned, x) >> 16);
}

__device__ __forceinline__ void relayout_split_elem(const float* __restrict__ w, int Cin, int Cout, int fl, int MT, long long total,
                                                    unsigned short* __restrict__ wr, int dgrad, long long e0, int max_slot, int nslot) {
  const int NP = npw_of(fl);
  float S = 1.0f;
  if (fl == 2) {
    unsigned mx = 0;
    for (int i = 0; i < nslot; ++i) mx = max(mx, reinterpret_cast<const unsigned*>(wr + total)[max_slot + i]);
    S = f16_weight_scale(__builtin_bit_cast(float, mx));
    if (e0 == 0) reinterpret_cast<float*>(wr + total)[0] = 1.0f / S;
  }
  if (e0 >= total) return;
  const int e = (int)(e0 & 7), row = (int)((e0 >> 3) & 31), half = (int)((e0 >> 8) & 1);
  long long r = e0 >> 9;
  const int mt = (int)(r % MT); r /= MT;
  const int pl = (int)(r % NP); r /= NP;
  const int dx = (int)(r % 3); r /= 3;
  const int dy = (int)(r % 3); r /= 3;
  const int nch = Cin / KC;
  const int chunk = (int)(r % nch);
  const int cb = (int)(r / nch);
  const int co = (cb * MT + mt) * 32 + row, ci = chunk * KC + 8 * half + e;
  float v = 0.0f;
  if (co < Cout) v = dgrad ? w[((size_t)ci * Cout + co) * 9 + (2 - dy) * 3 + (2 - dx)] : w[((size_t)co * Cin + ci) * 9 + dy * 3 + dx];
  wr[e0] = fl == 2 ? f16_piece(v, pl, S) : bf16_piece(v, pl, fl == 1);
}

__global__ void __launch_bounds__(256) conv3x3_relayout_split_kernel(const float* __restrict__ w, int Cin, int Cout, int fl, int MT,
                                                                      long long total, unsigned short* __restrict__ wr, int dgrad) {
  relayout_split_elem(w, Cin, Cout, fl, MT, total, wr, dgrad, (long long)blockIdx.x * 256 + threadIdx.x, 3, 1);
}

__device__ __forceinline__ unsigned absmax_wave(const float* __restrict__ w, long long n, long long first, long long stride) {
  unsigned m = 0;
  for (long long i = first; i < n; i += stride) m = max(m, __builtin_bit_cast(unsigned, w[i]) & 0x7fffffffu);
#pragma unroll
  for (int off = 32; off > 0; off >>= 1) m = max(m, (unsigned)__shfl_xor((int)m, off, 64));
  return m;
}
__global__ void __launch_bounds__(256) weight_absmax_kernel(const float* __restrict__ w, long long n, unsigned* __restrict__ slot) {
  const unsigned m = absmax_wave(w, n, (long long)blockIdx.x * 256 + threadIdx.x, (long long)gridDim.x * 256);
  if ((threadIdx.x & 63) == 0 && m) atomicMax(slot + 3, m);
}

constexpr int ABSMAX_SPLIT = 8;
__global__ void __launch_bounds__(256) weight_absmax_multi_kernel(const long long* __restrict__ jobs) {
  const long long* jb = jobs + (size_t)blockIdx.x * 8;
  if ((int)(jb[4] & 0xf) != 2) return;
  const long long n = jb[2] * jb[3] * 9;
  const unsigned m = absmax_wave(reinterpret_cast<const float*>(jb[0]), n, (long long)blockIdx.y * 256 + threadIdx.x, (long long)ABSMAX_SPLIT * 256);
  __shared__ unsigned part[4];
  if ((threadIdx.x & 63) == 0) part[threadIdx.x >> 6] = m;
  __syncthreads();
  if (threadIdx.x == 0)
    (reinterpret_cast<unsigned*>(reinterpret_cast<unsigned short*>(jb[1]) + jb[5]))[8 + blockIdx.y] = max(max(part[0], part[1]), max(part[2], part[3]));
}
__global__ void __launch_bounds__(256) conv3x3_relayout_split_multi_kernel(const long long* __restrict__ jobs, int njobs) {
  int lo = 0, hi = njobs - 1;
  while (lo < hi) {
    const int mid = (lo + hi + 1) >> 1;
    if (jobs[(size_t)mid * 8 + 6] <= (long long)blockIdx.x) lo = mid; else hi = mid - 1;
  }
  const long long* jb = jobs + (size_t)lo * 8;
  const int flags = (int)jb[4];
  relayout_split_elem(reinterpret_cast<const float*>(jb[0]), (int)jb[2], (int)jb[3], flags & 0xff, (flags >> 8) & 0xff, jb[5],
                      reinterpret_cast<unsigned short*>(jb[1]), (flags >> 16) & 1, ((long long)blockIdx.x - jb[6]) * 256 + threadIdx.x, 8,
                      ABSMAX_SPLIT);
}

template <int I, int N, class F>
__device__ __forceinline__ void static_for(F&& f) {
  if constexpr (I < N) {
    f(std::integral_constant<int, I>());
    static_for<I + 1, N>(f);
  }
}
template <int IMM>
__device__ __forceinline__ void lds_read128(bf16x8& d, unsigned addr) {
  asm volatile("ds_read_b128 %0, %1 offset:%2" : "=v"(d) : "v"(addr), "n"(IMM) : "memory");
// ... 589 lines not shown
                      };
                      if (p.res1) res(p.res1, (p.io_flags & 4) != 0);
                      if (p.res2) res(p.res2, (p.io_flags & 8) != 0);
                      *reinterpret_cast<f32x4*>(ob + mt * 32 + 8 * qd) = v;
                    }
                    continue;
                  }
                }
                if (co + 3 < p.Cout) {
                  if (p.res1) v += *reinterpret_cast<const f32x4*>(p.res1 + opix + co);
                  if (p.res2) v += *reinterpret_cast<const f32x4*>(p.res2 + opix + co);
                  *reinterpret_cast<f32x4*>(ob + mt * 32 + 8 * qd) = v;
                } else {
                  for (int e = 0; e < 4 && co + e < p.Cout; ++e) {
                    float sv = v[e];
                    if (p.res1) sv += p.res1[opix + co + e];
                    if (p.res2) sv += p.res2[opix + co + e];
                    ob[mt * 32 + 8 * qd + e] = sv;
                  }
                }
              }
          } else if constexpr (MODE == 1) {
            float* ob = p.out + (size_t)b * p.out_img_pitch + (size_t)(2 * y) * p.out_row_pitch +
                        (size_t)(2 * x) * p.out_pix_pitch + (co_e >> 2);
#pragma unroll
            for (int mt = 0; mt < MT; ++mt) {
              if (cb * MW + mt * 32 + 32 <= p.Cout && p.out_vec4 && !(p.io_flags & C2M_IO_DWORD_STORES)) {
#pragma unroll
                for (int e = 0; e < 4; ++e) {
                  const float q0 = acc[mt][nt][e], q1 = acc[mt][nt][4 + e], q2 = acc[mt][nt][8 + e], q3 = acc[mt][nt][12 + e];
                  const auto ra = __builtin_amdgcn_permlane32_swap(__builtin_bit_cast(unsigned, q0), __builtin_bit_cast(unsigned, q2), false, false);
                  const auto rb = __builtin_amdgcn_permlane32_swap(__builtin_bit_cast(unsigned, q1), __builtin_bit_cast(unsigned, q3), false, false);
                  const unsigned a0 = ra[0], a1 = ra[1], b0 = rb[0], b1 = rb[1];
                  const f32x4 v = {__builtin_bit_cast(float, a0), __builtin_bit_cast(float, a1), __builtin_bit_cast(float, b0), __builtin_bit_cast(float, b1)};
                  *reinterpret_cast<f32x4*>(ob + (size_t)(e >> 1) * p.out_row_pitch + (size_t)(e & 1) * p.out_pix_pitch + mt * 8 + 3 * hi) = v;
                }
                continue;
              }
#pragma unroll
              for (int qd = 0; qd < 4; ++qd)
                if (co_e + mt * 32 + 8 * qd < p.Cout) {
#pragma unroll
                  for (int e = 0; e < 4; ++e)
                    ob[(size_t)(e >> 1) * p.out_row_pitch + (size_t)(e & 1) * p.out_pix_pitch + mt * 8 + 2 * qd] = acc[mt][nt][4 * qd + e];
                }
            }
          } else {
            const size_t HWs = (size_t)p.H * p.W;
            if ((p.W & 3) == 0 && !(p.io_flags & C2M_IO_DWORD_STORES)) {
#pragma unroll
              for (int mt = 0; mt < MT; ++mt)
#pragma unroll
                for (int qd = 0; qd < 4; ++qd) {
                  f32x4 v;
#pragma unroll
                  for (int e = 0; e < 4; ++e) v[e] = acc[mt][nt][4 * qd + e];
                  const f32x4 t = quad_transpose(v, j);
                  const int ch = co_e + mt * 32 + 8 * qd + (j & 3);
                  if (ch < p.Cout) *reinterpret_cast<f32x4*>(p.out + ((size_t)b * p.Cout + ch) * HWs + (size_t)y * p.W + (x & ~3)) = t;
                }
              continue;
            }
            float* ob = p.out + ((size_t)b * p.Cout + co_e) * HWs + (size_t)y * p.W + x;
#pragma unroll
            for (int mt = 0; mt < MT; ++mt)
#pragma unroll
              for (int r = 0; r < 16; ++r) {
                const int cr = mt * 32 + 8 * (r >> 2) + (r & 3);
                if (co_e + cr < p.Cout) ob[(size_t)cr * HWs] = acc[mt][nt][r];
              }
          }
        }
      }
    }
#pragma unroll
    for (int mt = 0; mt < MT; ++mt)
#pragma unroll
      for (int nt = 0; nt < NT; ++nt)
#pragma unroll
        for (int r = 0; r < 16; ++r) acc[mt][nt][r] = 0.0f;
  }
  if constexpr (FL == 2) {
    if (p.range_flag != nullptr && !(amax < 65520.0f)) *p.range_flag = 1;
  }
}

}
}
}

using namespace c2m;

namespace c2m {
namespace conv {

static size_t split_image_bytes(int Cin, int Cout, int np) {
  if (Cin <= 0 || Cout <= 0 || Cin % split::KC != 0 || (np != 1 && np != 2 && np != 3)) return 0;
  const int MT = cout_tiles(Cout), ncb = (Cout + 32 * MT - 1) / (32 * MT);
  return (size_t)ncb * (Cin / split::KC) * 3 * 3 * split::npw_of(np) * MT * 1024;
}

size_t split_relayout_bytes(int Cin, int Cout, int np) {
  const size_t b = split_image_bytes(Cin, Cout, np);
  return b == 0 ? 0 : b + (np == 2 ? 256 : 0);
}

int split_relayout(hipStream_t st, const float* weight, int Cin, int Cout, int np, void* wr, int dgrad) {
  const size_t bytes = split_image_bytes(Cin, Cout, np);
  if (bytes == 0) return C2M_ERR_UNSUPPORTED;
  const long long total = (long long)(bytes / 2);
  if (np == 2) {
    const long long n = (long long)Cin * Cout * 9;
    (void)hipMemsetAsync(reinterpret_cast<char*>(wr) + bytes, 0, 256, st);
    hipLaunchKernelGGL(split::weight_absmax_kernel, dim3((unsigned)std::min<long long>(64, (n + 4095) / 4096)), dim3(256), 0, st, weight, n,
                       reinterpret_cast<unsigned*>(reinterpret_cast<char*>(wr) + bytes));
  }
  hipLaunchKernelGGL(split::conv3x3_relayout_split_kernel, dim3((unsigned)((total + 255) / 256)), dim3(256), 0, st, weight, Cin,
                     Cout, np, cout_tiles(Cout), total, reinterpret_cast<unsigned short*>(wr), dgrad);
  return check_launch();
}

int split_relayout_multi(hipStream_t st, const long long* jobs, int njobs, long long nblocks, int any_f16) {
  if (njobs <= 0 || nblocks <= 0 || nblocks > 0x7fffffffLL || !jobs) return C2M_ERR_INVALID_ARG;
  if (any_f16) hipLaunchKernelGGL(split::weight_absmax_multi_kernel, dim3((unsigned)njobs, split::ABSMAX_SPLIT), dim3(256), 0, st, jobs);
  hipLaunchKernelGGL(split::conv3x3_relayout_split_multi_kernel, dim3((unsigned)nblocks), dim3(256), 0, st, jobs, njobs);
  return check_launch();
}

template <int NP>
static int launch_split_mode(hipStream_t st, const Params& p, dim3 grid, int MT) {
  using split::conv3x3_split_kernel;
  struct Kernel { void (*fn)(Params); unsigned long long lds_done; };
  static Kernel kernels[2][6] = {
      {{&conv3x3_split_kernel<NP, 1, 0>, 0}, {&conv3x3_split_kernel<NP, 1, 1>, 0}, {&conv3x3_split_kernel<NP, 1, 2>, 0},
       {&conv3x3_split_kernel<NP, 1, 3>, 0}, {&conv3x3_split_kernel<NP, 1, 4>, 0}, {&conv3x3_split_kernel<NP, 1, 5>, 0}},
      {{&conv3x3_split_kernel<NP, 2, 0>, 0}, {&conv3x3_split_kernel<NP, 2, 1>, 0}, {&conv3x3_split_kernel<NP, 2, 2>, 0},
       {&conv3x3_split_kernel<NP, 2, 3>, 0}, {&conv3x3_split_kernel<NP, 2, 4>, 0}, {&conv3x3_split_kernel<NP, 2, 5>, 0}}};
  size_t ldsb = (size_t)((NP != 3 ? 2 : 1) * split::npx_of(NP) * 2 * split::HALFB) + (NP != 3 ? 3 : 2) * (size_t)(3 * split::npw_of(NP) * MT * 1024) + 1024 + 256;
  int mode = p.out_mode;
  if (mode == 3 && p.W % 4 == 0 && !(p.io_flags & C2M_IO_DWORD_STORES)) mode = 5;
  Kernel* k = &kernels[MT - 1][mode];
  if constexpr (NP == 1) {
    if (p.io_flags & C2M_IO_SRC_BF16) {
      static Kernel src16[2] = {{&conv3x3_split_kernel<1, 1, 0, true>, 0}, {&conv3x3_split_kernel<1, 2, 0, true>, 0}};
      k = &src16[MT - 1];
      ldsb = (size_t)3 * 12 * 1024 + 3 * (size_t)(3 * MT * 1024) + 1024 + 256;
    }
  }
  const int rc = ensure_dynamic_lds(reinterpret_cast<const void*>(k->fn), ldsb, k->lds_done);
  if (rc == C2M_OK) hipLaunchKernelGGL(k->fn, grid, dim3(256), ldsb, st, p);
  return rc;
}

int launch_split(hipStream_t st, Params p, int np) {
  p.tiles_x = ceil_div(p.W, split::TWX);
  p.tiles_y = ceil_div(p.H, split::THY);
  p.nchunks = p.Cin / split::KC;
  const int MT = cout_tiles(p.Cout), ncb = ceil_div(p.Cout, 32 * MT);
  const long long ntile = (long long)p.tiles_x * p.tiles_y * p.B;
  if (ntile > 0x7fffffffLL) return C2M_ERR_INVALID_ARG;
  p.tpw = tiles_per_workgroup(ntile, ncb, 512, 16);
  dim3 grid((unsigned)((ntile + p.tpw - 1) / p.tpw), ncb);
  const int rc = np == 3 ? launch_split_mode<3>(st, p, grid, MT) : np == 2 ? launch_split_mode<2>(st, p, grid, MT) : launch_split_mode<1>(st, p, grid, MT);
  if (rc != C2M_OK) return rc;
  return check_launch();
}

}
}
```

c2-matching_amd/mmsr/models/archs/contras_extractor_arch.py:

```python
import torch
import torch.nn as nn

from mmsr.models.archs.vgg_arch import NAMES, build_vgg_features


class ContrasExtractorLayer(nn.Module):

    def __init__(self):
        super().__init__()
        self.model = nn.Sequential(build_vgg_features('vgg16', NAMES['vgg16'].index('conv3_1')))
        self.register_buffer('mean', torch.Tensor([0.485, 0.456, 0.406]).view(1, 3, 1, 1))
        self.register_buffer('std', torch.Tensor([0.229, 0.224, 0.225]).view(1, 3, 1, 1))

    def forward(self, batch):
        from c2m_amd import ops as _ops
        if (not torch.is_grad_enabled() and batch.is_cuda and batch.dtype == torch.float32 and batch.shape[1] == 3 and
                (not torch.is_autocast_enabled('cuda') or _ops.bf16_autocast())):
            out = _ops.f16_range_guard(self, lambda: _ops.vgg_stack_forward(self.model._modules, batch, mean=self.mean, std=self.std,
                                                                              last_nchw=True), batch.device)
            return out['conv3_1']
        return self.model((batch - self.mean) / self.std)


class ContrasExtractorSep(nn.Module):

    def __init__(self):
        super().__init__()
        self.feature_extraction_image1 = ContrasExtractorLayer()
        self.feature_extraction_image2 = ContrasExtractorLayer()

    def forward(self, image1, image2):
        def both():
            return {'dense_features1': self.feature_extraction_image1(image1),
                    'dense_features2': self.feature_extraction_image2(image2)}
        if not torch.is_grad_enabled() and image1.is_cuda and image1.dtype == torch.float32:
            from c2m_amd import ops as _ops
            return _ops.f16_range_guard(self, both, image1.device)
        return both()
```

c2-matching_amd/mmsr/models/archs/corres_generation_arch.py:

```python
import logging

import torch
import torch.nn as nn

from c2m_amd import ops as _ops
from mmsr.models.archs.vgg_arch import VGGFeatureExtractor

logger = logging.getLogger('base')


class PreOffsets(dict):

    _SCALE = {'relu3_1': 1, 'relu2_1': 2, 'relu1_1': 4}

    def __init__(self, max_idx, h=None, w=None):
        super().__init__()
        if isinstance(max_idx, torch.Tensor):
            dict.__setitem__(self, 'max_idx', max_idx)
        else:
            for k, v in dict(max_idx).items():
                dict.__setitem__(self, k, v)
            if not dict.__contains__(self, 'max_idx'):
                raise TypeError("PreOffsets needs the arg-max index map (a tensor, or a mapping with key 'max_idx')")
        mi = dict.__getitem__(self, 'max_idx')
        self.h = int(h) if h is not None else mi.shape[-2] + 2
        self.w = int(w) if w is not None else mi.shape[-1] + 2
        self._flow = None

    @property
    def max_idx(self):
        return dict.__getitem__(self, 'max_idx')

    @property
    def flow(self):
        if self._flow is None:
            self._flow = _ops.index_to_flow(self.max_idx)
        return self._flow

    def __missing__(self, key):
        if key not in self._SCALE:
            raise KeyError(key)
        (t,) = _ops.build_pre_offsets(self.max_idx, self.h, self.w, scales=(self._SCALE[key],))
        dict.__setitem__(self, key, t)
        return t

    def __contains__(self, key):
        return key in self._SCALE or dict.__contains__(self, key)

    def get(self, key, default=None):
        return self[key] if key in self else default

    def __reduce__(self):
        return (type(self), (dict(self.items()), self.h, self.w))


class CorrespondenceGenerationArch(nn.Module):

    def __init__(self, patch_size=3, stride=1, vgg_layer_list=['relu3_1', 'relu2_1', 'relu1_1'], vgg_type='vgg19'):
        super(CorrespondenceGenerationArch, self).__init__()
        self.patch_size = patch_size
        self.stride = stride
        self.vgg_layer_list = vgg_layer_list
        self.vgg = VGGFeatureExtractor(layer_name_list=vgg_layer_list, vgg_type=vgg_type)
        self.vgg.grouped8_taps = ('relu1_1',)
        self.vgg.fast_conv = True

    def index_to_flow(self, max_idx):
        h, w = max_idx.shape
        (flow,) = _ops.build_pre_offsets(max_idx[None].contiguous(), h + 2, w + 2, scales=(1,))
        return flow[:, 0]

    @torch.no_grad()
    def match(self, dense_features):
        feat_in = _ops.feature_normalize(dense_features['dense_features1'].float(), with_sumsq=True)
        feat_ref = _ops.feature_normalize(dense_features['dense_features2'].float(), with_sumsq=True)
        return _ops.feature_match_index_batched(feat_in, feat_ref, self.patch_size, self.stride, self.stride,
                                                is_norm=True, norm_input=True)

    def forward(self, dense_features, img_ref_hr):
        if self.patch_size != 3 or self.stride != 1:
            raise NotImplementedError('pre-offset generation is defined for patch_size=3, stride=1')
        h, w = dense_features['dense_features1'].shape[2:]
        max_idx, _ = self.match(dense_features)
        pre_offset = PreOffsets(max_idx, h, w)
        img_ref_feat = self.vgg(img_ref_hr)
        return pre_offset, img_ref_feat
```

c2-matching_amd/mmsr/models/archs/vgg_arch.py:

```python
import logging
import os
import warnings
from collections import OrderedDict

import torch
import torch.nn as nn

logger = logging.getLogger('base')

_CFG = {
    'vgg11': [64, 'M', 128, 'M', 256, 256, 'M', 512, 512, 'M', 512, 512, 'M'],
    'vgg13': [64, 64, 'M', 128, 128, 'M', 256, 256, 'M', 512, 512, 'M', 512, 512, 'M'],
    'vgg16': [64, 64, 'M', 128, 128, 'M', 256, 256, 256, 'M', 512, 512, 512, 'M', 512, 512, 512, 'M'],
    'vgg19': [64, 64, 'M', 128, 128, 'M', 256, 256, 256, 256, 'M', 512, 512, 512, 512, 'M', 512, 512, 512, 512, 'M'],
}


def layer_names(vgg_type):
    names, block, idx = [], 1, 1
    for v in _CFG[vgg_type]:
        if v == 'M':
            names.append(f'pool{block}')
            block, idx = block + 1, 1
        else:
            names += [f'conv{block}_{idx}', f'relu{block}_{idx}']
            idx += 1
    return names


NAMES = {k: layer_names(k) for k in _CFG}


def build_vgg_features(vgg_type, upto, pretrained=True):
    names = NAMES[vgg_type][:upto + 1]
    tv_layers, local_state = None, None
    if pretrained:
        try:
            import torchvision.models.vgg as tv_vgg
        except ImportError:
            tv_vgg = None
        if tv_vgg is not None:
            enum = getattr(tv_vgg, f'{vgg_type.upper()}_Weights', None)
            net = getattr(tv_vgg, vgg_type)(weights=enum.IMAGENET1K_V1) if enum is not None else \
                getattr(tv_vgg, vgg_type)(pretrained=True)
            tv_layers = list(net.features[:upto + 1])
        else:
            path = os.path.join(os.environ.get('C2M_VGG_WEIGHTS', ''), f'{vgg_type}.pth')
            if os.environ.get('C2M_VGG_WEIGHTS') and os.path.exists(path):
                local_state = torch.load(path, map_location='cpu')
            else:
                msg = (f'torchvision is not installed and $C2M_VGG_WEIGHTS/{vgg_type}.pth was not found: the {vgg_type} '
                       'feature stack starts from RANDOM weights.  Load a checkpoint (or pass pretrained=False) before '
                       'using it on real images.')
                logger.warning(msg)
                warnings.warn(msg, RuntimeWarning, stacklevel=2)
    out, c_in, pos = OrderedDict(), 3, 0
    for v in _CFG[vgg_type]:
        n_here = 1 if v == 'M' else 2
        if pos >= len(names):
            break
        if v == 'M':
            out[names[pos]] = tv_layers[pos] if tv_layers else nn.MaxPool2d(kernel_size=2, stride=2)
        else:
            out[names[pos]] = tv_layers[pos] if tv_layers else nn.Conv2d(c_in, v, kernel_size=3, padding=1)
            if pos + 1 < len(names):
                out[names[pos + 1]] = tv_layers[pos + 1] if tv_layers else nn.ReLU(inplace=True)
            c_in = v
        pos += n_here
    if local_state is not None:
        for k, name in enumerate(names):
            if isinstance(out[name], nn.Conv2d):
                out[name].weight.data.copy_(local_state[f'features.{k}.weight'])
                out[name].bias.data.copy_(local_state[f'features.{k}.bias'])
    return out


def _bf16_autocast():
    from c2m_amd import ops as _ops
    return _ops.bf16_autocast()


class VGGFeatureExtractor(nn.Module):

    def __init__(self, layer_name_list, vgg_type='vgg19', use_input_norm=True, requires_grad=False,
                 remove_pooling=False, pooling_stride=2):
        super().__init__()
        if 'bn' in vgg_type:
            raise NotImplementedError('batch-norm VGG variants are not used by C2-Matching')
        self.layer_name_list = layer_name_list
        self.use_input_norm = use_input_norm
        self.names = NAMES[vgg_type]
        last = max(self.names.index(n) for n in layer_name_list)
        stack = OrderedDict()
        for name, layer in build_vgg_features(vgg_type, last).items():
            if 'pool' in name:
                if remove_pooling:
                    continue
                layer = nn.MaxPool2d(kernel_size=2, stride=pooling_stride)
            stack[name] = layer
        self.vgg_net = nn.Sequential(stack)
        if not requires_grad:
            for p in self.parameters():
                p.requires_grad = False
        if use_input_norm:
            self.register_buffer('mean', torch.Tensor([0.485, 0.456, 0.406]).view(1, 3, 1, 1))
            self.register_buffer('std', torch.Tensor([0.229, 0.224, 0.225]).view(1, 3, 1, 1))

    def _use_fused(self, x):
        def ok(m):
            if isinstance(m, nn.Conv2d):
                return (m.kernel_size == (3, 3) and m.stride == (1, 1) and m.padding == (1, 1) and m.groups == 1 and
                        (m.in_channels == 3 or m.in_channels % 32 == 0))
            if isinstance(m, nn.MaxPool2d):
                return m.kernel_size in (2, (2, 2)) and m.stride in (2, (2, 2))
            return isinstance(m, nn.ReLU)
        return (not torch.is_grad_enabled() and x.is_cuda and x.dtype == torch.float32 and x.dim() == 4 and x.shape[1] == 3 and
                (not torch.is_autocast_enabled('cuda') or _bf16_autocast()) and all(ok(m) for m in self.vgg_net._modules.values()) and
                all(n.startswith('relu') for n in self.layer_name_list))

    def forward(self, x):
        if self._use_fused(x):
            from c2m_amd import ops as _ops
            return _ops.f16_range_guard(self, lambda: _ops.vgg_stack_forward(
                self.vgg_net._modules, x, taps=self.layer_name_list, mean=self.mean if self.use_input_norm else None,
                std=self.std if self.use_input_norm else None, grouped8_taps=getattr(self, 'grouped8_taps', ()),
                fast=getattr(self, 'fast_conv', False)), x.device)
        if self.use_input_norm:
            x = (x - self.mean) / self.std
        taps = {}
        for name, layer in self.vgg_net._modules.items():
            x = layer(x)
            if name in self.layer_name_list:
                taps[name] = x.clone()
        return taps
```

c2-matching_amd/mmsr/models/ref_restoration_model.py:

```python
import collections
import copy
import logging
import os

import torch

import mmsr.models.networks as networks
from mmsr.models.base_model import BaseModel, unwrap
from mmsr.utils import metrics

logger = logging.getLogger('base')

_VAL_FUSED = os.environ.get("C2M_VAL_FUSED", "1") != "0"


class RefRestorationModel(BaseModel):

    def __init__(self, opt):
        super().__init__(opt)
        opt = copy.deepcopy(opt)
        self.net_g = self.model_to_device(networks.define_net_g(opt))
        self.net_map = self.model_to_device(networks.define_net_map(opt), receives_gradients=False)
        self.net_extractor = self.model_to_device(networks.define_net_extractor(opt), receives_gradients=False)
        for p in self.net_extractor.parameters():
# ... 53 lines not shown
            return
        self.img_in_lq = data['img_in_lq'].to(self.device)
        self.img_ref = data['img_ref'].to(self.device)
        self.gt = data['img_in'].to(self.device)
        self.match_img_in = data['img_in_up'].to(self.device)

    def _correspondence(self):
        with torch.no_grad():
            self.features = self.net_extractor(self.match_img_in, self.img_ref)
            self.pre_offset, self.img_ref_feat = self.net_map(self.features, self.img_ref)

    def optimize_parameters(self, step):
        if self._graph_on:
            return self._optimize_graphed()
        self._train_step()

    def _train_step(self):
        self._correspondence()
        self.output = self.net_g(self.img_in_lq, self.pre_offset, self.img_ref_feat)
        self.optimizer_g.zero_grad()
        l_pix = self.cri_pix(self.output, self.gt) * self.pixel_weight
        l_pix.backward()
        self.optimizer_g.step()
        self.log_dict['l_g_pix'] = l_pix.detach()

    GRAPH_WARMUP_STEPS = 2

    def _optimize_graphed(self):
        if self._graph is not None:
            self._graph.replay()
            self.output = self._graph_output
            return
        self._graph_calls += 1
        cur = torch.cuda.current_stream()
        if self._graph_calls <= self.GRAPH_WARMUP_STEPS:
            side = torch.cuda.Stream()
            side.wait_stream(cur)
            with torch.cuda.stream(side):
                self._train_step()
            cur.wait_stream(side)
            return
        self.optimizer_g.zero_grad(set_to_none=True)
        graph = torch.cuda.CUDAGraph()
        with torch.cuda.graph(graph):
            self._train_step()
        self._graph = graph
        self._graph_output = self.output
        graph.replay()

    def get_current_visuals(self):
        shown = [('img_in_lq', self.img_in_lq), ('rlt', self.output)] + ([('gt', self.gt)] if hasattr(self, 'gt') else [])
        return collections.OrderedDict((k, t.detach().cpu()) for k, t in shown)

    def _save_img_path(self, img_name, dataset_name, current_iter):
        root = (self.opt.get('path') or {}).get('visualization')
        if not root:
            raise ValueError("save_img needs opt['path']['visualization'] (the directory the images go to)")
        if self.opt.get('is_train'):
            return os.path.join(root, img_name, f'{img_name}_{current_iter}.png')
        stem = f"{img_name}_{self.opt.get('name')}"
        if self.opt.get('suffix'):
            stem += f"_{self.opt['suffix']}"
        return os.path.join(root, dataset_name, stem + '.png')

    @staticmethod
    def _img_names(val_data, idx, count):
        paths = val_data.get('lq_path')
        if isinstance(paths, str):
            paths = [paths]
        names = [os.path.splitext(os.path.basename(p_))[0] for p_ in (paths or [])][:count]
        for b in range(len(names), count):
            names.append(str(idx) if count == 1 else f'{idx}_{b}')
        return names

    @staticmethod
    def _write_png(rgb_u8, path):
        try:
            from PIL import Image
        except ImportError as e:
            raise RuntimeError("save_img=True writes PNG files with Pillow, which is not installed "
                               "(pip install pillow), or validate with save_img=False") from e
        os.makedirs(os.path.dirname(path), exist_ok=True)
        Image.fromarray(rgb_u8.contiguous().numpy(), 'RGB').save(path)

    @staticmethod
    def _fused_validation(sr, gt):
        return bool(_VAL_FUSED and sr.is_cuda and gt.is_cuda and sr.dtype == torch.float32 and gt.dtype == torch.float32)

    def _validate_shard(self, dataloader, rank, world, save=None):
        crop = self.opt.get('crop_border')
        crop = self.opt.get('scale', 4) if crop is None else crop
        sums = torch.zeros(4, dtype=torch.float64, device=self.device)
        for idx, val_data in enumerate(dataloader):
            if idx % world != rank:
                continue
            self._eval_feed = True
            try:
                self.feed_data(val_data)
            finally:
                self._eval_feed = False
            sr = self.test()
            gt = self.gt
            valid = None
            if val_data.get('padding', False) is not False and bool(torch.as_tensor(val_data['padding']).any()):
                valid = tuple(int(torch.as_tensor(v).flatten()[0]) for v in val_data['original_size'][:2])
            if self._fused_validation(sr, gt):
                m = metrics.validation_metrics_fused(sr, gt, crop_border=crop, valid_hw=valid, images='rgb' if save else None)
                rgb = m['sr_u8'] if save else None
            else:
                if valid is not None:
                    sr, gt = sr[..., :valid[0], :valid[1]], gt[..., :valid[0], :valid[1]]
                with metrics.true_scalar_division():
                    m = metrics.validation_metrics(sr, gt, crop_border=crop)
                rgb = metrics.tensor2img_device(sr).flip(-1).to(torch.uint8) if save else None
            if save:
                rgb = rgb.cpu()
                for b, img_name in enumerate(self._img_names(val_data, idx, rgb.shape[0])):
                    self._write_png(rgb[b], self._save_img_path(img_name, save[0], save[1]))
            sums[0] += m['psnr'].sum()
            sums[1] += m['psnr_y'].sum()
            sums[2] += m['ssim_y'].sum()
            sums[3] += sr.shape[0]
            del self.img_in_lq, self.output, self.gt
        return sums

    def _report(self, sums, name, current_iter, tb_logger):
        n = max(float(sums[3]), 1.0)
        res = {'psnr': float(sums[0]) / n, 'psnr_y': float(sums[1]) / n, 'ssim_y': float(sums[2]) / n, 'count': int(sums[3])}
        if self.rank <= 0:
            logger.info(f"# Validation {name} # PSNR: {res['psnr']:.4e} # PSNR_Y: {res['psnr_y']:.4e} "
                        f"# SSIM_Y: {res['ssim_y']:.4e}.")
            if tb_logger:
                for k in ('psnr', 'psnr_y', 'ssim_y'):
                    tb_logger.add_scalar(k, res[k], current_iter)
        return res

    def nondist_validation(self, dataloader, current_iter, tb_logger, save_img):
        name = getattr(getattr(dataloader, 'dataset', None), 'opt', {}).get('name', 'val')
        sums = self._validate_shard(dataloader, 0, 1, save=(name, current_iter) if save_img else None)
        return self._report(sums, name, current_iter, tb_logger)

    def dist_validation(self, dataloader, current_iter, tb_logger, save_img):
        import torch.distributed as dist
        rank, world = dist.get_rank(), dist.get_world_size()
        name = getattr(getattr(dataloader, 'dataset', None), 'opt', {}).get('name', 'val')
        sums = self._validate_shard(dataloader, rank, world, save=(name, current_iter) if save_img else None)
        dist.all_reduce(sums, op=dist.ReduceOp.SUM)
        return self._report(sums, name, current_iter, tb_logger)

    def test(self):
        self.net_g.eval()
        with torch.no_grad():
            def whole():
                self._correspondence()
                return self.net_g(self.img_in_lq, self.pre_offset, self.img_ref_feat)
            if self.img_in_lq.is_cuda:
                from c2m_amd import ops as _ops
                self.output = _ops.f16_range_guard(self, whole, self.img_in_lq.device)
            else:
                self.output = whole()
        if self.is_train:
            self.net_g.train()
        return self.output
```

include/c2m_hip.h:

```cpp
#ifndef C2M_HIP_H
#define C2M_HIP_H

#include <stddef.h>
#include <stdint.h>

#ifdef __cplusplus
extern "C" {
#endif

typedef void* c2m_stream_t;

typedef enum c2m_status {
  C2M_OK = 0,
  C2M_ERR_INVALID_ARG = 1,
  C2M_ERR_UNSUPPORTED = 2,
  C2M_ERR_WORKSPACE = 3,
  C2M_ERR_LAUNCH = 4,
  C2M_ERR_NO_DEVICE = 5
} c2m_status;

int c2m_abi_version(void);
const char* c2m_status_string(int status);
const char* c2m_last_hip_error(void);
int c2m_device_arch(char* buf, int buflen);

enum { C2M_KERNEL_CORR_MFMA = 1, C2M_KERNEL_CORR_GENERIC = 2, C2M_KERNEL_DCN_FWD = 3, C2M_KERNEL_DCN_BWD_DATA = 4,
       C2M_KERNEL_DCN_BWD_WEIGHT = 5, C2M_KERNEL_CONV3X3 = 6 ,
       C2M_KERNEL_CONV3X3_SPLIT = 7 ,
       C2M_KERNEL_CONV3X3_WGRAD = 8,
       C2M_KERNEL_CORR_FILTER = 9 ,
       C2M_KERNEL_CORR_RESOLVE = 10  };
enum { C2M_ACT_NONE = 0, C2M_ACT_RELU = 1, C2M_ACT_LEAKY_RELU = 2 };
int c2m_profile_enable(int on);
int c2m_profile_collect(float* ms, int* kernel_id, int capacity, int* count);


int c2m_feature_normalize_f32(c2m_stream_t stream, const float* x, int B, int C, int HW, float* out);
int c2m_feature_normalize_ss_f32(c2m_stream_t stream, const float* x, int B, int C, int HW, float* out, float* ss_out);

size_t c2m_feature_match_workspace_bytes(int B, int Hq, int Wq, int Hr, int Wr);
size_t c2m_feature_match_workspace_bytes_c(int B, int C, int Hq, int Wq, int Hr, int Wr);

int c2m_feature_match_skip_table(int B, int Hq, int Wq, int Hr, int Wr, size_t* byte_offset, int* x_tiles);

int c2m_feature_match_filter_tables(int B, int Hq, int Wq, int Hr, int Wr, size_t* cnt_offset, size_t* cand_offset,
                                    size_t* flags_offset, int* slots);

#define C2M_CORR_FORCE_GENERIC 1
#define C2M_CORR_EXACT_SWEEP 2
int c2m_feature_match_index_f32(c2m_stream_t stream, const float* feat_in, const float* feat_ref, int B, int C,
                                int Hq, int Wq, int Hr, int Wr, int patch, int in_stride, int ref_stride,
                                int is_norm, int norm_input, int flags, int64_t* max_idx, float* max_val,
                                void* workspace, size_t workspace_bytes);
int c2m_feature_match_index_pre_f32(c2m_stream_t stream, const float* feat_in, const float* feat_ref, int B, int C,
                                    int Hq, int Wq, int Hr, int Wr, int patch, int in_stride, int ref_stride,
                                    int is_norm, int norm_input, int flags, int64_t* max_idx, float* max_val,
                                    void* workspace, size_t workspace_bytes, const float* ss_in_pre, const float* ss_ref_pre);

int c2m_build_pre_offsets_f32(c2m_stream_t stream, const int64_t* max_idx, int B, int h, int w, float* off3,
                              float* off2, float* off1);

size_t c2m_dcn_v2_forward_workspace_bytes(int B, int C, int H, int W, int Co, int kh, int kw, int dg);
int c2m_dcn_v2_forward_f32(c2m_stream_t stream, const float* input, const float* weight, const float* bias,
                           const float* offset, const float* mask, int B, int C, int H, int W, int Co, int kh, int kw,
                           int sh, int sw, int ph, int pw, int dh, int dw, int dg, float* output, void* workspace,
                           size_t workspace_bytes);

int c2m_dcn_v2_forward_bf16mma_f32(c2m_stream_t stream, const float* input, const float* weight, const float* bias,
                                   const float* offset, const float* mask, int B, int C, int H, int W, int Co, int kh,
                                   int kw, int sh, int sw, int ph, int pw, int dh, int dw, int dg, float* output,
                                   void* workspace, size_t workspace_bytes);

int c2m_nchw_to_nhwc_bordered_f32(c2m_stream_t stream, const float* input, int B, int C, int H, int W, float* out);
size_t c2m_dcn_v2_relayout_bytes(int C, int Co, int kh, int kw, int dg);
int c2m_dcn_v2_relayout_f32(c2m_stream_t stream, const float* weight, int C, int Co, int kh, int kw, int dg, float* wt);
int c2m_dcn_v2_forward_nhwc_f32(c2m_stream_t stream, const float* input_bordered, const float* wt, const float* bias,
                                const float* offset, const float* mask, int B, int C, int H, int W, int Co, int kh, int kw,
                                int sh, int sw, int ph, int pw, int dh, int dw, int dg, float* output, int out_nhwc,
                                int out_pix_pitch, int out_row_pitch, long long out_img_pitch, int act, float slope,
                                int input_grouped);

size_t c2m_dcn_v2_relayout_f16x2_bytes(int C, int Co, int kh, int kw, int dg);
int c2m_dcn_v2_relayout_f16x2(c2m_stream_t stream, const float* weight, int C, int Co, int kh, int kw, int dg, void* wt);
int c2m_dcn_v2_forward_nhwc_f16x2(c2m_stream_t stream, const float* input_bordered, const void* wt, const float* bias,
                                  const float* offset, const float* mask, int B, int C, int H, int W, int Co, int kh, int kw,
                                  int sh, int sw, int ph, int pw, int dh, int dw, int dg, float* output, int out_nhwc,
                                  int out_pix_pitch, int out_row_pitch, long long out_img_pitch, int act, float slope,
                                  int input_grouped, int* range_flag);

size_t c2m_dcn_v2_backward_workspace_bytes(int B, int C, int H, int W, int Co, int kh, int kw, int sh, int sw, int ph,
                                           int pw, int dh, int dw, int dg);
int c2m_dcn_v2_backward_f32(c2m_stream_t stream, const float* input, const float* weight, const float* bias,
                            const float* offset, const float* mask, const float* grad_output, int B, int C, int H,
                            int W, int Co, int kh, int kw, int sh, int sw, int ph, int pw, int dh, int dw, int dg,
                            float* grad_input, float* grad_offset, float* grad_mask, float* grad_weight,
                            float* grad_bias, void* workspace, size_t workspace_bytes);

#define C2M_ABS_SUM_SLOTS 256
int c2m_dcn_fuse_offsets_f32(c2m_stream_t stream, const float* conv_out, const float* pre_offset, int B, int dg, int K,
                             int H, int W, float* offset, float* mask, double* abs_sum);

typedef struct c2m_conv_src {
  const float* ptr;
  int C;
  int pix_pitch;
  int row_pitch;
  long long img_pitch;
} c2m_conv_src;

enum { C2M_CONV_DIRECT = 0, C2M_CONV_WINOGRAD_F23X = 1, C2M_CONV_WINOGRAD_F43X = 2, C2M_CONV_SPLIT_BF16X3 = 3, C2M_CONV_BF16 = 4,
       C2M_CONV_SPLIT_F16X2 = 5 };
enum { C2M_OUT_NHWC = 0, C2M_OUT_NHWC_PIXEL_SHUFFLE2 = 1, C2M_OUT_NCHW = 2, C2M_OUT_DCN_HEAD = 3, C2M_OUT_NHWC_MAXPOOL2 = 4 };

typedef struct c2m_conv3x3_desc {
  int B, H, W, Cin, Cout;
  int nsrc;
  c2m_conv_src src[2];
  const float* wr;
  const float* bias;
  int act;
  float slope;
  int out_mode;
  float* out;
  int out_pix_pitch, out_row_pitch;
  long long out_img_pitch;
  const float* res1;
  const float* res2;
  float* mask_out;
  const float* flow;
  int fh, fw;
  int scale;
  int n_off;
  double* abs_sum;
  int algo;
  int cout_offset;
  int cout_total;
  float* out2;
  int out2_row_pitch;
  long long out2_plane_pitch, out2_img_pitch;
  int* range_flag;
  int io_flags;
} c2m_conv3x3_desc;
#define C2M_IO_SRC_BF16 1
#define C2M_IO_OUT_BF16 2
#define C2M_IO_RES1_BF16 4
#define C2M_IO_RES2_BF16 8
#define C2M_IO_DWORD_STORES 16

size_t c2m_conv3x3_relayout_bytes(int Cin, int Cout);
int c2m_conv3x3_relayout_f32(c2m_stream_t stream, const float* weight , int Cin, int Cout, float* wr);
size_t c2m_conv3x3_relayout_wino_bytes(int Cin, int Cout);
int c2m_conv3x3_relayout_wino_f32(c2m_stream_t stream, const float* weight, int Cin, int Cout, float* wr);
size_t c2m_conv3x3_relayout_wino4_bytes(int Cin, int Cout);
int c2m_conv3x3_relayout_wino4_f32(c2m_stream_t stream, const float* weight, int Cin, int Cout, float* wr);
size_t c2m_conv3x3_relayout_split_bytes(int Cin, int Cout, int pieces);
int c2m_conv3x3_relayout_split_f32(c2m_stream_t stream, const float* weight, int Cin, int Cout, int pieces, void* wr);
int c2m_conv3x3_relayout_split_multi(c2m_stream_t stream, const long long* jobs, int njobs, long long nblocks, int any_f16);
int c2m_conv3x3_nhwc_f32(c2m_stream_t stream, const c2m_conv3x3_desc* desc);

int c2m_conv3x3_relayout_split_dgrad_f32(c2m_stream_t stream, const float* weight , int Cin, int Cout,
                                         int pieces, void* wr);
size_t c2m_conv3x3_wgrad_workspace_bytes(int B, int H, int W, int Cin, int Cout);
int c2m_conv3x3_wgrad_f32(c2m_stream_t stream, const c2m_conv_src* src, int nsrc, const float* grad_out, int g_pix_pitch,
                          int g_row_pitch, long long g_img_pitch, int B, int H, int W, int Cin, int Cout, float* grad_weight,
                          void* workspace, size_t workspace_bytes);

int c2m_conv3x3_rgb64_f32(c2m_stream_t stream, const float* image, int B, int H, int W, const float* weight,
                          const float* bias, const float* mean, const float* std_, int act, float slope, float* out,
                          int out_pix_pitch, int out_row_pitch, long long out_img_pitch, float* out2, int out2_row_pitch,
                          long long out2_plane_pitch, long long out2_img_pitch);

int c2m_index_to_flow_f32(c2m_stream_t stream, const int64_t* max_idx, int B, int hq, int wq, float* flow);

size_t c2m_contras_loss_workspace_bytes(int B, int C, int H1, int W1, int Ntot, int with_teacher);
int c2m_contras_loss_forward_f32(c2m_stream_t stream, const float* f1, const float* f2, const float* tf1, const float* tf2,
                                 int B, int C, int H1, int W1, int H2, int W2, const int* ids, const int* pos2,
                                 const int* offsets, int Ntot, int max_n, float margin, float safe_radius,
                                 float temperature, float* out, void* workspace, size_t workspace_bytes);
int c2m_contras_loss_backward_f32(c2m_stream_t stream, int B, int C, int H1, int W1, int H2, int W2, const int* ids,
                                  const int* pos2, const int* offsets, int Ntot, int max_n, float margin,
                                  float safe_radius, float temperature, int with_teacher, const float* grad_terms,
                                  float* grad_f1, float* grad_f2, void* workspace, size_t workspace_bytes);

int c2m_contras_loss_rows_f32(c2m_stream_t stream, int B, int C, int H1, int W1, int Ntot, int with_teacher,
                              const void* workspace, size_t workspace_bytes, float* pos, float* neg1, int* neg1_idx,
                              float* neg2, int* neg2_idx);

int c2m_warp_perspective_u8(c2m_stream_t stream, const uint8_t* src, const double* M, const double* M_inv, int B, int H,
                            int W, float* dst_f32, uint8_t* dst_u8, double* coords);
int c2m_pil_bicubic_u8(c2m_stream_t stream, const uint8_t* src, int N, int H, int W, int vertical, int out_size,
                       const int* start, const int* count, const int* coeff, int K, uint8_t* dst_u8, float* dst_f32);

#define C2M_PIL2D_TILE 32
#define C2M_PIL2D_LDS_BUDGET 65536
size_t c2m_pil_bicubic2d_lds_bytes(int Kh, int Kv, int win_h, int win_w);
int c2m_pil_bicubic2d_u8(c2m_stream_t stream, const uint8_t* src, const uint8_t* flags, int N, int planes_per_sample, int H,
                         int W, int out_h, int out_w, const int* h_start, const int* h_count, const int* h_coeff, int Kh,
                         const int* v_start, const int* v_count, const int* v_coeff, int Kv, int win_h, int win_w,
                         uint8_t* dst_u8, float* dst_f32, float* orient_f32);

typedef struct c2m_image_src {
  const float* ptr;
  long long pix_pitch;
  long long row_pitch, plane_pitch, img_pitch;
} c2m_image_src;
#define C2M_VAL_TILE_H 16
#define C2M_VAL_TILE_W 32
int c2m_val_metrics_tile(int* tile_h, int* tile_w);
size_t c2m_val_metrics_workspace_bytes(int B, int valid_h, int valid_w, int crop_border);
int c2m_val_metrics_f32(c2m_stream_t stream, const c2m_image_src* sr, const c2m_image_src* gt, int B, int H, int W,
                        int valid_h, int valid_w, int crop_border, int rgb_order, uint8_t* sr_u8, uint8_t* gt_u8,
                        double* sums, void* workspace, size_t workspace_bytes);

#ifdef __cplusplus
}
#endif
#endif
```

Before: 116.8.

## Skip VGG conv tiles over zero-padded Ref regions and fill them from a template

```diff
diff --git a/c2-matching_amd/c2m_amd/_lib.py b/c2-matching_amd/c2m_amd/_lib.py
--- a/c2-matching_amd/c2m_amd/_lib.py
+++ b/c2-matching_amd/c2m_amd/_lib.py
@@ -93,6 +93,12 @@
     L.c2m_conv3x3_wgrad_workspace_bytes.argtypes = [_i] * 5
     L.c2m_conv3x3_wgrad_f32.argtypes = [_vp, ctypes.POINTER(ConvSrc), _i, _vp, _i, _i, ctypes.c_longlong] + [_i] * 5 + [_vp, _vp, _sz]
     L.c2m_conv3x3_nhwc_f32.argtypes = [_vp, ctypes.POINTER(Conv3x3Desc)]
+    L.c2m_conv3x3_nhwc_roi_f32.argtypes = [_vp, ctypes.POINTER(Conv3x3Desc), _i, _i]
+    L.c2m_conv3x3_rgb64_roi_f32.argtypes = L.c2m_conv3x3_rgb64_f32.argtypes + [_i, _i]
+    L.c2m_conv3x3_roi_tile.argtypes = [_i, ctypes.POINTER(_i), ctypes.POINTER(_i)]
+    L.c2m_ref_live_extent_f32.argtypes = [_vp, _vp, _i, _i, _i, _vp]
+    _ll = ctypes.c_longlong
+    L.c2m_band_fill_f32.argtypes = [_vp, _vp, _i, _i, _i, _i, _i, _i, _i, _ll, _ll, _vp, _i, _i, _i, _i, _ll] + [_i] * 5
     L.c2m_index_to_flow_f32.argtypes = [_vp, _vp, _i, _i, _i, _vp]
     L.c2m_contras_loss_workspace_bytes.restype = _sz
     L.c2m_contras_loss_workspace_bytes.argtypes = [_i] * 6
diff --git a/c2-matching_amd/c2m_amd/ops.py b/c2-matching_amd/c2m_amd/ops.py
--- a/c2-matching_amd/c2m_amd/ops.py
+++ b/c2-matching_amd/c2m_amd/ops.py
@@ -553,6 +553,16 @@
 
 
 def f16_range_guard(owner, fn, device):
+    if getattr(_tls, "live_cache", None) is not None:
+        return _f16_range_guard(owner, fn, device)
+    _tls.live_cache = {}
+    try:
+        return _f16_range_guard(owner, fn, device)
+    finally:
+        _tls.live_cache = None
+
+
+def _f16_range_guard(owner, fn, device):
     if getattr(_tls, "guarded", False):
         return fn()
     if getattr(owner, "_c2m_conv_bf16x3", False):
@@ -637,16 +647,28 @@
     return o
 
 
-def _launch_conv(d, dev, kind, family_prefix=""):
+def _roi_pixels(roi_tiles, H, W, rgb64=False):
+    if roi_tiles is None:
+        return H, W
+    th, tw = conv_roi_tile(rgb64)
+    return min(roi_tiles[0] * th, H), min(roi_tiles[1] * tw, W)
+
+
+def _launch_conv(d, dev, kind, family_prefix="", roi_tiles=None):
     with torch.cuda.device(dev):
-        _lib.check(_lib.lib().c2m_conv3x3_nhwc_f32(_stream(), d), "c2m_conv3x3_nhwc_f32")
+        if roi_tiles is None:
+            _lib.check(_lib.lib().c2m_conv3x3_nhwc_f32(_stream(), d), "c2m_conv3x3_nhwc_f32")
+        else:
+            _lib.check(_lib.lib().c2m_conv3x3_nhwc_roi_f32(_stream(), d, int(roi_tiles[0]), int(roi_tiles[1])),
+                       "c2m_conv3x3_nhwc_roi_f32")
     if _ConvFlops.enabled:
-        f = 2.0 * d.Cout * 9 * d.Cin * d.H * d.W * d.B
+        rh, rw = _roi_pixels(roi_tiles, d.H, d.W)
+        f = 2.0 * d.Cout * 9 * d.Cin * rh * rw * d.B
         _ConvFlops.add(family_prefix + _KINDS[kind].family, f, f * _KINDS[kind].exec_factor)
 
 
 def conv3x3(srcs, weight, bias=None, act=ACT_NONE, slope=0.1, res1=None, res2=None, out_mode="nhwc", out=None, algo=None,
-            out2_grouped8=None, fast=False, out_dtype=None, dword_stores=False):
+            out2_grouped8=None, fast=False, out_dtype=None, dword_stores=False, roi_tiles=None):
     srcs = _as_list(srcs)
     B, _, H, W = srcs[0].shape
     Cin = sum(s.shape[1] for s in srcs)
@@ -721,7 +743,9 @@
         d.out = out.data_ptr()
     else:
         raise _lib.C2MError(f"unknown out_mode {out_mode}")
-    _launch_conv(d, dev, kind)
+    if roi_tiles is not None and kind not in _SPLIT_KINDS:
+        raise _lib.C2MError("conv3x3: roi_tiles needs one of the split kernels")
+    _launch_conv(d, dev, kind, roi_tiles=roi_tiles)
     return out
 
 
@@ -825,7 +849,8 @@
     return g2.data_ptr() + ((W + 3) + 1) * 8 * 4, (W + 3) * 8, (H + 3) * (W + 3) * 8, (Cout // 8) * (H + 3) * (W + 3) * 8
 
 
-def conv3x3_rgb64(image, weight, bias=None, act=ACT_NONE, slope=0.1, mean=None, std=None, out=None, out2_grouped8=None):
+def conv3x3_rgb64(image, weight, bias=None, act=ACT_NONE, slope=0.1, mean=None, std=None, out=None, out2_grouped8=None,
+                  roi_tiles=None):
     if image.dim() != 4 or image.shape[1] != 3 or not image.is_cuda:
         raise _lib.C2MError("conv3x3_rgb64: image must be a GPU tensor [B,3,H,W]")
     if tuple(weight.shape) != (64, 3, 3, 3):
@@ -847,14 +872,18 @@
     if tuple(out.shape) != (B, 64, H, W):
         raise _lib.C2MError("conv3x3_rgb64: out must be [B,64,H,W]")
     o2, o2_row, o2_plane, o2_img = _grouped8_args(out2_grouped8, B, 64, H, W, dev)
+    args = (x.data_ptr(), B, H, W, w.data_ptr(), bias.data_ptr() if bias is not None else None,
+            mean.data_ptr() if mean is not None else None, std.data_ptr() if std is not None else None, int(act),
+            float(slope), out.data_ptr(), o.pix_pitch, o.row_pitch, o.img_pitch, o2, o2_row, o2_plane, o2_img)
     with torch.cuda.device(dev):
-        _lib.check(_lib.lib().c2m_conv3x3_rgb64_f32(
-            _stream(), x.data_ptr(), B, H, W, w.data_ptr(), bias.data_ptr() if bias is not None else None,
-            mean.data_ptr() if mean is not None else None, std.data_ptr() if std is not None else None, int(act),
-            float(slope), out.data_ptr(), o.pix_pitch, o.row_pitch, o.img_pitch, o2, o2_row, o2_plane, o2_img),
-            "c2m_conv3x3_rgb64_f32")
+        if roi_tiles is None:
+            _lib.check(_lib.lib().c2m_conv3x3_rgb64_f32(_stream(), *args), "c2m_conv3x3_rgb64_f32")
+        else:
+            _lib.check(_lib.lib().c2m_conv3x3_rgb64_roi_f32(_stream(), *args, int(roi_tiles[0]), int(roi_tiles[1])),
+                       "c2m_conv3x3_rgb64_roi_f32")
     if _ConvFlops.enabled:
-        _ConvFlops.add("rgb_first_layer", 2.0 * 64 * 27 * H * W * B, 2.0 * 64 * 28 * H * W * B)
+        rh, rw = _roi_pixels(roi_tiles, H, W, rgb64=True)
+        _ConvFlops.add("rgb_first_layer", 2.0 * 64 * 27 * rh * rw * B, 2.0 * 64 * 28 * rh * rw * B)
     return out
 
 
@@ -1023,6 +1052,173 @@
     return out
 
 
+_ref_band_on = True
+
+
+class ref_band_mode:
+
+    def __init__(self, mode):
+        self.mode = int(mode)
+        if self.mode not in (0, 1):
+            raise _lib.C2MError("ref_band_mode: 0 or 1")
+
+    def __enter__(self):
+        global _ref_band_on
+        self.prev, _ref_band_on = _ref_band_on, self.mode == 1
+        return self
+
+    def __exit__(self, *exc):
+        global _ref_band_on
+        _ref_band_on = self.prev
+        return False
+
+
+def conv_roi_tile(rgb64=False):
+    th, tw = ctypes.c_int(0), ctypes.c_int(0)
+    _lib.check(_lib.lib().c2m_conv3x3_roi_tile(int(bool(rgb64)), ctypes.byref(th), ctypes.byref(tw)), "c2m_conv3x3_roi_tile")
+    return th.value, tw.value
+
+
+def band_src_index(v, n, t, margin):
+    return v if v < margin else (t - (n - v) if n - v <= margin else margin)
+
+
+def stack_geometry(layers):
+    return ["conv" if isinstance(m, torch.nn.Conv2d) else "pool" for m in layers.values()
+            if isinstance(m, (torch.nn.Conv2d, torch.nn.MaxPool2d))]
+
+
+def ref_band_plan(geometry, H, W, live_h, live_w, first_rgb64=True, tiles=None):
+    if tiles is None:
+        tiles = (conv_roi_tile(True), conv_roi_tile(False))
+    n_pool = sum(1 for g in geometry if g == "pool")
+    if live_h is None or live_w is None or H % (1 << n_pool) != 0 or W % (1 << n_pool) != 0 or (live_h >= H and live_w >= W):
+        return None
+    convs, s, R, any_saved = [], 1, 0, False
+    for k, g in enumerate(geometry):
+        if g == "pool":
+            s *= 2
+            continue
+        R += s
+        th, tw = tiles[0] if (k == 0 and first_rgb64) else tiles[1]
+        Hc, Wc = H // s, W // s
+        full = (-(-Hc // th), -(-Wc // tw))
+        ext = (-(-(live_h + R) // s), -(-(live_w + R) // s))
+        roi = (max(1, min(full[0], -(-ext[0] // th))), max(1, min(full[1], -(-ext[1] // tw))))
+        any_saved |= roi != full
+        convs.append({"scale": s, "radius": R, "extent": ext, "tile": (th, tw), "tiles": full, "roi": roi})
+    if not convs or not any_saved:
+        return None
+    align = 4 * s
+    th, tw = tiles[1]
+    Ht = -(-(2 * R + 2 * s * th) // align) * align
+    Wt = -(-(2 * R + 2 * s * tw) // align) * align
+    for c in convs:
+        for sc in (c["scale"], 2 * c["scale"]):
+            m = band_margin(c["radius"], sc)
+            if min(H // sc, W // sc, Ht // sc, Wt // sc) < 2 * m + 1:
+                return None
+    return {"convs": convs, "template": (Ht, Wt)}
+
+
+def band_margin(radius, scale):
+    return -(-radius // scale) + 1
+
+
+def ref_live_extent(img):
+    if not img.is_cuda or img.dim() != 4 or img.shape[1] != 3 or img.dtype != torch.float32 or not img.is_contiguous():
+        raise _lib.C2MError("ref_live_extent: a contiguous float32 GPU tensor [B,3,H,W]")
+    B, _, H, W = img.shape
+    ext = torch.zeros(2, dtype=torch.int32, device=img.device)
+    with torch.cuda.device(img.device):
+        _lib.check(_lib.lib().c2m_ref_live_extent_f32(_stream(), img.data_ptr(), B, H, W, ext.data_ptr()), "c2m_ref_live_extent_f32")
+    lh, lw = ext.tolist()
+    return int(lh), int(lw)
+
+
+def ref_live_extent_shared(img):
+    if (not _ref_band_on or not isinstance(img, torch.Tensor) or not img.is_cuda or img.dim() != 4 or img.shape[1] != 3 or
+            img.dtype != torch.float32 or not img.is_contiguous() or img.numel() >= 2 ** 31 or
+            torch.cuda.is_current_stream_capturing()):
+        return None
+    cache = getattr(_tls, "live_cache", None)
+    key = (img.data_ptr(), tuple(img.shape), img._version, img.device)
+    if cache is not None and key in cache:
+        return cache[key]
+    live = ref_live_extent(img)
+    if cache is not None:
+        cache[key] = live
+    return live
+
+
+def band_fill(dst, tmpl, roi_h, roi_w, margin_y, margin_x, layout="nhwc"):
+    L = _lib.lib()
+    if layout == "grouped8":
+        B, G, Hb, Wb, e = dst.shape
+        _, Gt, Htb, Wtb, et = tmpl.shape
+        if e != 8 or et != 8 or G != Gt or not dst.is_contiguous() or not tmpl.is_contiguous() or tmpl.shape[0] != 1:
+            raise _lib.C2MError("band_fill: grouped8 buffers are contiguous [B, C/8, H+3, W+3, 8]")
+        H, W, Ht, Wt = Hb - 3, Wb - 3, Htb - 3, Wtb - 3
+        args = (dst.data_ptr() + (Wb + 1) * 32, B, G * 8, H, W, 8, 8, Wb * 8, Hb * Wb * 8, G * Hb * Wb * 8,
+                tmpl.data_ptr() + (Wtb + 1) * 32, Ht, Wt, 8, Wtb * 8, Htb * Wtb * 8)
+        planar = 0
+    elif layout == "nhwc":
+        B, C, H, W = dst.shape
+        Ht, Wt = tmpl.shape[2:]
+        d, t = _nhwc_src(dst, "dst"), _nhwc_src(tmpl, "tmpl")
+        if tmpl.shape[0] != 1 or tmpl.shape[1] != C:
+            raise _lib.C2MError("band_fill: the template is [1, C, Ht, Wt]")
+        args = (dst.data_ptr(), B, C, H, W, C, d.pix_pitch, d.row_pitch, 0, d.img_pitch,
+                tmpl.data_ptr(), Ht, Wt, t.pix_pitch, t.row_pitch, 0)
+        planar = 0
+    elif layout == "nchw":
+        B, C, H, W = dst.shape
+        Ht, Wt = tmpl.shape[2:]
+        if not dst.is_contiguous() or not tmpl.is_contiguous() or tuple(tmpl.shape[:2]) != (1, C):
+            raise _lib.C2MError("band_fill: nchw tensors are contiguous, the template [1, C, Ht, Wt]")
+        args = (dst.data_ptr(), B, C, H, W, 1, 0, 0, 0, 0, tmpl.data_ptr(), Ht, Wt, 0, 0, 0)
+        planar = 1
+    else:
+        raise _lib.C2MError(f"band_fill: unknown layout {layout}")
+    if dst.dtype != torch.float32 or tmpl.dtype != torch.float32 or not dst.is_cuda or tmpl.device != dst.device:
+        raise _lib.C2MError("band_fill: float32 GPU tensors on one device")
+    with torch.cuda.device(dst.device):
+        _lib.check(L.c2m_band_fill_f32(_stream(), *args, int(roi_h), int(roi_w), int(margin_y), int(margin_x), planar),
+                   "c2m_band_fill_f32")
+    return dst
+
+
+class _RefBand:
+
+    def __init__(self, plan, H, W, dev, algo):
+        self.plan, self.H, self.W, self.algo, self.k = plan, H, W, algo, 0
+        self.tcur = torch.zeros((1, 3) + tuple(plan["template"]), dtype=torch.float32, device=dev)
+
+    def conv(self, call, first, src, cout, out_mode, out, out2):
+        c = self.plan["convs"][self.k]
+        self.k += 1
+        extra = {} if first else {"algo": self.algo}
+        t2 = None
+        if out2 is not None:
+            t2 = torch.empty((1, cout // 8, self.tcur.shape[2] + 3, self.tcur.shape[3] + 3, 8), dtype=torch.float32, device=src.device)
+        t_out = call(self.tcur, None, t2, **extra)
+        self.tcur = t_out
+        if c["roi"] == c["tiles"]:
+            return call(src, out, out2, **extra)
+        res = call(src, out, out2, roi_tiles=c["roi"], **extra)
+        pooled = out_mode == "nhwc_pool2"
+        so = c["scale"] * (2 if pooled else 1)
+        Hc, Wc = self.H // c["scale"], self.W // c["scale"]
+        roi_h, roi_w = min(c["roi"][0] * c["tile"][0], Hc), min(c["roi"][1] * c["tile"][1], Wc)
+        if pooled:
+            roi_h, roi_w = roi_h // 2, roi_w // 2
+        m = band_margin(c["radius"], so)
+        band_fill(res, t_out, roi_h, roi_w, m, m, layout="nchw" if out_mode == "nchw" else "nhwc")
+        if out2 is not None:
+            band_fill(out2, t2, roi_h, roi_w, m, m, layout="grouped8")
+        return res
+
+
 def _bordered_empty(B, C, H, W, device, grouped8=False):
     def zero_border(t):
         t[..., 0, :, :].zero_()
@@ -1050,7 +1246,12 @@
     return two(m.kernel_size) and two(m.stride) and m.padding in (0, (0, 0)) and m.dilation in (1, (1, 1)) and not m.ceil_mode
 
 
-def vgg_stack_forward(layers, x, taps=(), mean=None, std=None, last_nchw=False, grouped8_taps=(), fast=False):
+def _band_split_ok(layer, fast):
+    co, ci = layer.weight.shape[:2]
+    return (_SPLIT == "all" or ((fast or bf16_autocast()) and _SPLIT != "0")) and ci % 16 == 0 and co % 4 == 0
+
+
+def vgg_stack_forward(layers, x, taps=(), mean=None, std=None, last_nchw=False, grouped8_taps=(), fast=False, live=None):
     names = list(layers.keys())
     B, C, H, W = x.shape
     dev = x.device
@@ -1066,12 +1267,27 @@
             xin = (xin - mean) / std
         cur[:, :C] = xin
     out, k = {}, 0
-
-    def conv(k_, src, layer_, **kw):
-        if k_ == 0 and rgb64:
-            kw.pop("algo", None)
-            return conv3x3_rgb64(src, layer_.weight, layer_.bias, mean=mean, std=std, **kw)
-        return conv3x3(src, layer_.weight, layer_.bias, fast=fast, **kw)
+    band = None
+    convs_ = [m for m in layers.values() if isinstance(m, torch.nn.Conv2d)]
+    if (live is not None and rgb64 and x.dtype == torch.float32 and
+            all(isinstance(m, (torch.nn.Conv2d, torch.nn.ReLU)) or (isinstance(m, torch.nn.MaxPool2d) and _pool_is_2x2(m))
+                for m in layers.values()) and
+            all(m.kernel_size == (3, 3) and m.stride == (1, 1) and m.padding == (1, 1) and m.groups == 1 for m in convs_) and
+            all(_band_split_ok(m, fast) for m in convs_[1:])):
+        plan = ref_band_plan(stack_geometry(layers), H, W, live[0], live[1])
+        if plan is not None:
+            band = _RefBand(plan, H, W, dev, _KINDS[_split_kind(None)].name)
+
+    def conv(k_, src, layer_, act=ACT_NONE, out_mode="nhwc", out=None, out2_grouped8=None):
+        first = k_ == 0 and rgb64
+
+        def call(src_, out_, out2_, **kw):
+            if first:
+                return conv3x3_rgb64(src_, layer_.weight, layer_.bias, act=act, mean=mean, std=std, out=out_, out2_grouped8=out2_, **kw)
+            return conv3x3(src_, layer_.weight, layer_.bias, act=act, out_mode=out_mode, out=out_, out2_grouped8=out2_, fast=fast, **kw)
+        if band is None:
+            return call(src, out, out2_grouped8)
+        return band.conv(call, first, src, layer_.out_channels, out_mode, out, out2_grouped8)
 
     while k < len(names):
         name, layer = names[k], layers[names[k]]
@@ -1089,7 +1305,7 @@
                     Hc % 2 == 0 and Wc % 2 == 0 and
                     (_wino_ok([cur], layer.weight, "nhwc_pool2", Wc) or _split_ok([cur], layer.weight, fast)))
             if last and last_nchw:
-                cur = conv3x3(cur, layer.weight, layer.bias, act=ACT_RELU if relu else ACT_NONE, out_mode="nchw", fast=fast)
+                cur = conv(-1, cur, layer, act=ACT_RELU if relu else ACT_NONE, out_mode="nchw")
                 out[names[k + 1] if relu else name] = cur
             elif tap_name is not None:
                 bo = _bordered_empty(Bc, layer.out_channels, Hc, Wc, dev, grouped8=tap_name in grouped8_taps)
@@ -1099,16 +1315,20 @@
                 out[tap_name] = view
                 cur = view
             elif pool:
-                cur = conv3x3(cur, layer.weight, layer.bias, act=ACT_RELU, out_mode="nhwc_pool2", fast=fast)
+                cur = conv(k, cur, layer, act=ACT_RELU, out_mode="nhwc_pool2")
                 k += 1
             else:
                 cur = conv(k, cur, layer, act=ACT_RELU if relu else ACT_NONE)
             k += 2 if relu else 1
         elif isinstance(layer, torch.nn.MaxPool2d):
             cur = torch.nn.functional.max_pool2d(cur, layer.kernel_size, layer.stride, layer.padding)
+            if band is not None:
+                band.tcur = torch.nn.functional.max_pool2d(band.tcur, layer.kernel_size, layer.stride, layer.padding)
             k += 1
         elif isinstance(layer, torch.nn.ReLU):
             cur = torch.relu(cur)
+            if band is not None:
+                band.tcur = torch.relu(band.tcur)
             k += 1
         else:
             raise _lib.C2MError(f"vgg_stack_forward: unsupported layer {name}: {type(layer).__name__}")
diff --git a/c2-matching_amd/csrc/conv3x3.hip b/c2-matching_amd/csrc/conv3x3.hip
--- a/c2-matching_amd/csrc/conv3x3.hip
+++ b/c2-matching_amd/csrc/conv3x3.hip
@@ -1222,7 +1222,7 @@
 namespace conv {
 size_t split_relayout_bytes(int Cin, int Cout, int np);
 int split_relayout(hipStream_t st, const float* weight, int Cin, int Cout, int np, void* wr, int dgrad);
-int launch_split(hipStream_t st, Params p, int np);
+int launch_split(hipStream_t st, Params p, int np, int roi_tiles_y = 0, int roi_tiles_x = 0);
 int split_relayout_multi(hipStream_t st, const long long* jobs, int njobs, long long nblocks, int any_f16);
 }
 }
@@ -1295,10 +1295,11 @@
   return check_launch();
 }
 
-extern "C" int c2m_conv3x3_rgb64_f32(c2m_stream_t stream, const float* image, int B, int H, int W, const float* weight,
-                                     const float* bias, const float* mean, const float* std_, int act, float slope, float* out,
-                                     int out_pix_pitch, int out_row_pitch, long long out_img_pitch, float* out2,
-                                     int out2_row_pitch, long long out2_plane_pitch, long long out2_img_pitch) {
+static int conv3x3_rgb64_launch(c2m_stream_t stream, const float* image, int B, int H, int W, const float* weight,
+                                const float* bias, const float* mean, const float* std_, int act, float slope, float* out,
+                                int out_pix_pitch, int out_row_pitch, long long out_img_pitch, float* out2,
+                                int out2_row_pitch, long long out2_plane_pitch, long long out2_img_pitch, int roi_tiles_y,
+                                int roi_tiles_x) {
   if (!image || !weight || !out || B <= 0 || H <= 0 || W <= 0 || (mean == nullptr) != (std_ == nullptr)) return C2M_ERR_INVALID_ARG;
   if (act < 0 || act > 2 || (act == C2M_ACT_LEAKY_RELU && !(slope >= 0.0f && slope <= 1.0f))) return C2M_ERR_UNSUPPORTED;
   if (out_pix_pitch % 4 != 0 || out_row_pitch % 4 != 0 || out_img_pitch % 4 != 0 || ((uintptr_t)out & 15)) return C2M_ERR_UNSUPPORTED;
@@ -1308,6 +1309,10 @@
   p.in = image; p.w = weight; p.bias = bias; p.mean = mean; p.std_ = std_;
   p.B = B; p.H = H; p.W = W;
   p.tiles_x = ceil_div(W, conv::c3::CTW); p.tiles_y = ceil_div(H, conv::c3::CTH);
+  if (roi_tiles_y > 0 && roi_tiles_x > 0) {
+    if (roi_tiles_y > p.tiles_y || roi_tiles_x > p.tiles_x) return C2M_ERR_INVALID_ARG;
+    p.tiles_y = roi_tiles_y; p.tiles_x = roi_tiles_x;
+  }
   p.act = act; p.slope = slope; p.out = out; p.out_pix_pitch = out_pix_pitch; p.out_row_pitch = out_row_pitch;
   p.out_img_pitch = out_img_pitch; p.out2 = out2; p.out2_row_pitch = out2_row_pitch; p.out2_plane_pitch = out2_plane_pitch;
   p.out2_img_pitch = out2_img_pitch;
@@ -1327,6 +1332,31 @@
   return check_launch();
 }
 
+extern "C" int c2m_conv3x3_rgb64_f32(c2m_stream_t stream, const float* image, int B, int H, int W, const float* weight,
+                                     const float* bias, const float* mean, const float* std_, int act, float slope, float* out,
+                                     int out_pix_pitch, int out_row_pitch, long long out_img_pitch, float* out2,
+                                     int out2_row_pitch, long long out2_plane_pitch, long long out2_img_pitch) {
+  return conv3x3_rgb64_launch(stream, image, B, H, W, weight, bias, mean, std_, act, slope, out, out_pix_pitch, out_row_pitch,
+                              out_img_pitch, out2, out2_row_pitch, out2_plane_pitch, out2_img_pitch, 0, 0);
+}
+
+extern "C" int c2m_conv3x3_rgb64_roi_f32(c2m_stream_t stream, const float* image, int B, int H, int W, const float* weight,
+                                         const float* bias, const float* mean, const float* std_, int act, float slope,
+                                         float* out, int out_pix_pitch, int out_row_pitch, long long out_img_pitch, float* out2,
+                                         int out2_row_pitch, long long out2_plane_pitch, long long out2_img_pitch,
+                                         int roi_tiles_y, int roi_tiles_x) {
+  if (roi_tiles_y <= 0 || roi_tiles_x <= 0) return C2M_ERR_INVALID_ARG;
+  return conv3x3_rgb64_launch(stream, image, B, H, W, weight, bias, mean, std_, act, slope, out, out_pix_pitch, out_row_pitch,
+                              out_img_pitch, out2, out2_row_pitch, out2_plane_pitch, out2_img_pitch, roi_tiles_y, roi_tiles_x);
+}
+
+extern "C" int c2m_conv3x3_roi_tile(int rgb64, int* tile_h, int* tile_w) {
+  if (!tile_h || !tile_w) return C2M_ERR_INVALID_ARG;
+  *tile_h = rgb64 ? conv::c3::CTH : conv::kSplitTileH;
+  *tile_w = rgb64 ? conv::c3::CTW : conv::kSplitTileW;
+  return C2M_OK;
+}
+
 extern "C" int c2m_index_to_flow_f32(c2m_stream_t stream, const int64_t* max_idx, int B, int hq, int wq, float* flow) {
   if (!max_idx || !flow || B <= 0 || hq <= 0 || wq <= 0) return C2M_ERR_INVALID_ARG;
   const int n = B * hq * wq;
@@ -1335,7 +1365,7 @@
   return check_launch();
 }
 
-extern "C" int c2m_conv3x3_nhwc_f32(c2m_stream_t stream, const c2m_conv3x3_desc* d) {
+static int conv3x3_nhwc_launch(c2m_stream_t stream, const c2m_conv3x3_desc* d, int roi_tiles_y, int roi_tiles_x) {
   if (!d || !d->wr || !d->out || d->B <= 0 || d->H <= 0 || d->W <= 0 || d->Cin <= 0 || d->Cout <= 0 || d->nsrc < 1 ||
       d->nsrc > 2 || !d->src[0].ptr || (d->nsrc == 2 && !d->src[1].ptr))
     return C2M_ERR_INVALID_ARG;
@@ -1343,6 +1373,7 @@
   const bool wino = d->algo == C2M_CONV_WINOGRAD_F23X || wino4;
   const bool splitk = d->algo == C2M_CONV_SPLIT_BF16X3 || d->algo == C2M_CONV_BF16 || d->algo == C2M_CONV_SPLIT_F16X2;
   if (d->algo != 0 && !wino && !splitk) return C2M_ERR_INVALID_ARG;
+  if (roi_tiles_y > 0 && !splitk) return C2M_ERR_UNSUPPORTED;
   if (splitk && (d->out2 || (d->out_mode == 4 && (d->H % 2 != 0 || d->W % 2 != 0 || d->res1 || d->res2)))) return C2M_ERR_UNSUPPORTED;
   if (wino && ((d->out_mode != 0 && d->out_mode != 3 && d->out_mode != 4) || d->Cout % 64 != 0 || d->W % 32 != 0)) return C2M_ERR_UNSUPPORTED;
   if (d->out_mode == 4 && !splitk && (d->algo != C2M_CONV_WINOGRAD_F23X || d->H % 2 != 0 || d->res1 || d->res2 || d->out2)) return C2M_ERR_UNSUPPORTED;
@@ -1419,7 +1450,8 @@
   }
   if (splitk) {
     ProfileScope prof(C2M_KERNEL_CONV3X3_SPLIT, as_stream(stream));
-    return conv::launch_split(as_stream(stream), p, d->algo == C2M_CONV_BF16 ? 1 : (d->algo == C2M_CONV_SPLIT_F16X2 ? 2 : 3));
+    return conv::launch_split(as_stream(stream), p, d->algo == C2M_CONV_BF16 ? 1 : (d->algo == C2M_CONV_SPLIT_F16X2 ? 2 : 3),
+                              roi_tiles_y, roi_tiles_x);
   }
   const int ncb = ceil_div(d->Cout, MW);
   p.tpw = conv::tiles_per_workgroup(ntile, ncb, wino4 ? 256 : 512, 10);
@@ -1444,3 +1476,10 @@
   hipLaunchKernelGGL(k.fn, grid, dim3(256), lds, st, p);
   return check_launch();
 }
+
+extern "C" int c2m_conv3x3_nhwc_f32(c2m_stream_t stream, const c2m_conv3x3_desc* d) { return conv3x3_nhwc_launch(stream, d, 0, 0); }
+
+extern "C" int c2m_conv3x3_nhwc_roi_f32(c2m_stream_t stream, const c2m_conv3x3_desc* d, int roi_tiles_y, int roi_tiles_x) {
+  if (roi_tiles_y <= 0 || roi_tiles_x <= 0) return C2M_ERR_INVALID_ARG;
+  return conv3x3_nhwc_launch(stream, d, roi_tiles_y, roi_tiles_x);
+}
diff --git a/c2-matching_amd/csrc/conv3x3_shared.h b/c2-matching_amd/csrc/conv3x3_shared.h
--- a/c2-matching_amd/csrc/conv3x3_shared.h
+++ b/c2-matching_amd/csrc/conv3x3_shared.h
@@ -46,6 +46,8 @@
 
 inline int cout_tiles(int Cout) { return Cout <= 32 ? 1 : 2; }
 
+constexpr int kSplitTileW = 32, kSplitTileH = 8;
+
 inline int tiles_per_workgroup(long long ntile, int ncb, long long resident, int tmax) {
   static const int env_tpw = [] { const char* e = getenv("C2M_CONV_TPW"); return e ? atoi(e) : 0; }();
   if (env_tpw > 0) return env_tpw;
diff --git a/c2-matching_amd/csrc/conv3x3_split.hip b/c2-matching_amd/csrc/conv3x3_split.hip
--- a/c2-matching_amd/csrc/conv3x3_split.hip
+++ b/c2-matching_amd/csrc/conv3x3_split.hip
@@ -17,6 +17,7 @@
 constexpr int KC = 16;
 constexpr int TWX = 32, THY = 8;
 constexpr int HWc = TWX + 2, HHr = THY + 2;
+static_assert(TWX == kSplitTileW && THY == kSplitTileH, "c2m_conv3x3_roi_tile reports the split kernels' tile");
 constexpr int NPIX = HWc * HHr;
 constexpr int NRAW_W = (NPIX * 4 + 255) / 256;
 constexpr int HALFB = NPIX * 16;
@@ -912,9 +913,14 @@
   return rc;
 }
 
-int launch_split(hipStream_t st, Params p, int np) {
+int launch_split(hipStream_t st, Params p, int np, int roi_tiles_y, int roi_tiles_x) {
   p.tiles_x = ceil_div(p.W, split::TWX);
   p.tiles_y = ceil_div(p.H, split::THY);
+  if (roi_tiles_y > 0 && roi_tiles_x > 0) {
+    if (roi_tiles_y > p.tiles_y || roi_tiles_x > p.tiles_x) return C2M_ERR_INVALID_ARG;
+    p.tiles_y = roi_tiles_y;
+    p.tiles_x = roi_tiles_x;
+  }
   p.nchunks = p.Cin / split::KC;
   const int MT = cout_tiles(p.Cout), ncb = ceil_div(p.Cout, 32 * MT);
   const long long ntile = (long long)p.tiles_x * p.tiles_y * p.B;
diff --git a/c2-matching_amd/csrc/ref_band.hip b/c2-matching_amd/csrc/ref_band.hip
--- /dev/null
+++ b/c2-matching_amd/csrc/ref_band.hip
@@ -0,0 +1,171 @@
+#include <algorithm>
+
+#include "c2m_common.h"
+
+namespace c2m {
+namespace {
+
+constexpr int kThreads = 256;
+
+__global__ void __launch_bounds__(kThreads) live_extent_kernel(const float* __restrict__ img, unsigned n, unsigned H, unsigned Wv,
+                                                               int vec, int* __restrict__ out) {
+  int my = 0, mx = 0;
+  const unsigned stride = gridDim.x * kThreads;
+  for (unsigned i = blockIdx.x * kThreads + threadIdx.x; i < n; i += stride) {
+    int last = -1;
+    if (vec == 4) {
+      const f32x4 v = *reinterpret_cast<const f32x4*>(img + 4 * (size_t)i);
+#pragma unroll
+      for (int e = 0; e < 4; ++e)
+        if (v[e] != 0.0f) last = e;
+    } else if (img[i] != 0.0f) {
+      last = 0;
+    }
+    if (last >= 0) {
+      const unsigned row = i / Wv, xv = i - row * Wv;
+      my = max(my, (int)(row % H) + 1);
+      mx = max(mx, (int)xv * vec + last + 1);
+    }
+  }
+#pragma unroll
+  for (int s = kWave / 2; s > 0; s >>= 1) {
+    my = max(my, __shfl_xor(my, s, kWave));
+    mx = max(mx, __shfl_xor(mx, s, kWave));
+  }
+  __shared__ int wy[kThreads / kWave], wx[kThreads / kWave];
+  if ((threadIdx.x & (kWave - 1)) == 0) {
+    wy[threadIdx.x / kWave] = my;
+    wx[threadIdx.x / kWave] = mx;
+  }
+  __syncthreads();
+  if (threadIdx.x == 0) {
+#pragma unroll
+    for (int w = 1; w < kThreads / kWave; ++w) {
+      my = max(my, wy[w]);
+      mx = max(mx, wx[w]);
+    }
+    if (my > *(volatile int*)out) atomicMax(out, my);
+    if (mx > *(volatile int*)(out + 1)) atomicMax(out + 1, mx);
+  }
+}
+
+struct FillParams {
+  float* dst;
+  const float* tmpl;
+  int B, C, H, W, Ht, Wt;
+  int cpg;
+  int d_pix, d_row;
+  long long d_plane, d_img;
+  int t_pix, t_row;
+  long long t_plane;
+  int roi_h, roi_w, margin_y, margin_x;
+  long long n_a, n_band;
+};
+
+__device__ __forceinline__ int band_src(int v, int N, int T, int margin) {
+  return v < margin ? v : (N - v <= margin ? T - (N - v) : margin);
+}
+
+__device__ __forceinline__ void band_pixel(const FillParams& p, long long q, int wq, int rq, int& y, int& x) {
+  if (q < p.n_a) {
+    const int wa = wq - rq;
+    y = (int)(q / wa);
+    x = rq + (int)(q - (long long)y * wa);
+  } else {
+    q -= p.n_a;
+    y = p.roi_h + (int)(q / wq);
+    x = (int)(q - (long long)(y - p.roi_h) * wq);
+  }
+}
+
+__global__ void __launch_bounds__(kThreads) band_fill_vec_kernel(FillParams p) {
+  const int cv = p.C >> 2;
+  const long long per_img = p.n_band * cv;
+  const long long i = (long long)blockIdx.x * kThreads + threadIdx.x;
+  if (i >= per_img * p.B) return;
+  const int b = (int)(i / per_img);
+  const long long r = i - (long long)b * per_img;
+  const long long q = r / cv;
+  const int c = 4 * (int)(r - q * cv);
+  int y, x;
+  band_pixel(p, q, p.W, p.roi_w, y, x);
+  const int sy = band_src(y, p.H, p.Ht, p.margin_y), sx = band_src(x, p.W, p.Wt, p.margin_x);
+  const int plane = c / p.cpg, ci = c - plane * p.cpg;
+  const f32x4 v = *reinterpret_cast<const f32x4*>(p.tmpl + (size_t)plane * p.t_plane + (size_t)sy * p.t_row + (size_t)sx * p.t_pix + ci);
+  *reinterpret_cast<f32x4*>(p.dst + (size_t)b * p.d_img + (size_t)plane * p.d_plane + (size_t)y * p.d_row + (size_t)x * p.d_pix + ci) = v;
+}
+
+__global__ void __launch_bounds__(kThreads) band_fill_planar_kernel(FillParams p) {
+  const long long per_img = p.n_band * p.C;
+  const long long i = (long long)blockIdx.x * kThreads + threadIdx.x;
+  if (i >= per_img * p.B) return;
+  const int b = (int)(i / per_img);
+  const long long r = i - (long long)b * per_img;
+  const int c = (int)(r / p.n_band);
+  const long long q = r - (long long)c * p.n_band;
+  int y, xq;
+  band_pixel(p, q, p.W >> 2, p.roi_w >> 2, y, xq);
+  const int sy = band_src(y, p.H, p.Ht, p.margin_y);
+  const float* trow = p.tmpl + ((size_t)c * p.Ht + sy) * p.Wt;
+  f32x4 v;
+#pragma unroll
+  for (int e = 0; e < 4; ++e) v[e] = trow[band_src(4 * xq + e, p.W, p.Wt, p.margin_x)];
+  *reinterpret_cast<f32x4*>(p.dst + (((size_t)b * p.C + c) * p.H + y) * p.W + 4 * xq) = v;
+}
+
+}
+}
+
+extern "C" int c2m_ref_live_extent_f32(c2m_stream_t stream, const float* img, int B, int H, int W, int* extent) {
+  using namespace c2m;
+  if (!img || !extent || B <= 0 || H <= 0 || W <= 0) return C2M_ERR_INVALID_ARG;
+  const int vec = (W % 4 == 0 && ((uintptr_t)img & 15) == 0) ? 4 : 1;
+  const long long n = 3LL * B * H * W / vec;
+  if (n >= (1LL << 31)) return C2M_ERR_UNSUPPORTED;
+  const unsigned grid = (unsigned)std::min<long long>((n + kThreads - 1) / kThreads, 2048);
+  hipLaunchKernelGGL(live_extent_kernel, dim3(grid), dim3(kThreads), 0, as_stream(stream), img, (unsigned)n, (unsigned)H,
+                     (unsigned)(W / vec), vec, extent);
+  return check_launch();
+}
+
+extern "C" int c2m_band_fill_f32(c2m_stream_t stream, float* dst, int B, int C, int H, int W, int cpg, int d_pix_pitch,
+                                 int d_row_pitch, long long d_plane_pitch, long long d_img_pitch, const float* tmpl, int Ht,
+                                 int Wt, int t_pix_pitch, int t_row_pitch, long long t_plane_pitch, int roi_h, int roi_w,
+                                 int margin_y, int margin_x, int planar) {
+  using namespace c2m;
+  if (!dst || !tmpl || B <= 0 || C <= 0 || H <= 0 || W <= 0 || Ht <= 0 || Wt <= 0 || roi_h < 0 || roi_w < 0 || roi_h > H ||
+      roi_w > W || margin_y < 0 || margin_x < 0)
+    return C2M_ERR_INVALID_ARG;
+  if (H < 2 * margin_y + 1 || Ht < 2 * margin_y + 1 || W < 2 * margin_x + 1 || Wt < 2 * margin_x + 1) return C2M_ERR_INVALID_ARG;
+  if (((uintptr_t)dst & 15) || ((uintptr_t)tmpl & 15)) return C2M_ERR_UNSUPPORTED;
+  FillParams p;
+  p.dst = dst; p.tmpl = tmpl; p.B = B; p.C = C; p.H = H; p.W = W; p.Ht = Ht; p.Wt = Wt;
+  p.roi_h = roi_h; p.roi_w = roi_w; p.margin_y = margin_y; p.margin_x = margin_x;
+  long long threads;
+  if (planar) {
+    if (W % 4 != 0 || roi_w % 4 != 0) return C2M_ERR_UNSUPPORTED;
+    p.cpg = 1; p.d_pix = 1; p.d_row = W; p.d_plane = (long long)H * W; p.d_img = p.d_plane * C;
+    p.t_pix = 1; p.t_row = Wt; p.t_plane = (long long)Ht * Wt;
+    p.n_a = (long long)roi_h * ((W - roi_w) / 4);
+    p.n_band = p.n_a + (long long)(H - roi_h) * (W / 4);
+    threads = p.n_band * C * B;
+  } else {
+    if (cpg <= 0 || cpg % 4 != 0 || C % cpg != 0 || d_pix_pitch < cpg || t_pix_pitch < cpg || d_pix_pitch % 4 != 0 ||
+        d_row_pitch % 4 != 0 || d_plane_pitch % 4 != 0 || d_img_pitch % 4 != 0 || t_pix_pitch % 4 != 0 || t_row_pitch % 4 != 0 ||
+        t_plane_pitch % 4 != 0 || d_row_pitch < 0 || t_row_pitch < 0 || d_plane_pitch < 0 || t_plane_pitch < 0 || d_img_pitch < 0)
+      return C2M_ERR_UNSUPPORTED;
+    p.cpg = cpg; p.d_pix = d_pix_pitch; p.d_row = d_row_pitch; p.d_plane = d_plane_pitch; p.d_img = d_img_pitch;
+    p.t_pix = t_pix_pitch; p.t_row = t_row_pitch; p.t_plane = t_plane_pitch;
+    p.n_a = (long long)roi_h * (W - roi_w);
+    p.n_band = p.n_a + (long long)(H - roi_h) * W;
+    threads = p.n_band * (C / 4) * B;
+  }
+  if (threads == 0) return C2M_OK;
+  const long long blocks = (threads + kThreads - 1) / kThreads;
+  if (blocks > 0x7fffffffLL) return C2M_ERR_UNSUPPORTED;
+  if (planar)
+    hipLaunchKernelGGL(band_fill_planar_kernel, dim3((unsigned)blocks), dim3(kThreads), 0, as_stream(stream), p);
+  else
+    hipLaunchKernelGGL(band_fill_vec_kernel, dim3((unsigned)blocks), dim3(kThreads), 0, as_stream(stream), p);
+  return check_launch();
+}
diff --git a/c2-matching_amd/mmsr/models/archs/contras_extractor_arch.py b/c2-matching_amd/mmsr/models/archs/contras_extractor_arch.py
--- a/c2-matching_amd/mmsr/models/archs/contras_extractor_arch.py
+++ b/c2-matching_amd/mmsr/models/archs/contras_extractor_arch.py
@@ -12,12 +12,12 @@
         self.register_buffer('mean', torch.Tensor([0.485, 0.456, 0.406]).view(1, 3, 1, 1))
         self.register_buffer('std', torch.Tensor([0.229, 0.224, 0.225]).view(1, 3, 1, 1))
 
-    def forward(self, batch):
+    def forward(self, batch, live=None):
         from c2m_amd import ops as _ops
         if (not torch.is_grad_enabled() and batch.is_cuda and batch.dtype == torch.float32 and batch.shape[1] == 3 and
                 (not torch.is_autocast_enabled('cuda') or _ops.bf16_autocast())):
             out = _ops.f16_range_guard(self, lambda: _ops.vgg_stack_forward(self.model._modules, batch, mean=self.mean, std=self.std,
-                                                                              last_nchw=True), batch.device)
+                                                                              last_nchw=True, live=live), batch.device)
             return out['conv3_1']
         return self.model((batch - self.mean) / self.std)
 
@@ -29,11 +29,16 @@
         self.feature_extraction_image1 = ContrasExtractorLayer()
         self.feature_extraction_image2 = ContrasExtractorLayer()
 
+    ref_band = True
+
     def forward(self, image1, image2):
-        def both():
+        def both(live=None):
             return {'dense_features1': self.feature_extraction_image1(image1),
-                    'dense_features2': self.feature_extraction_image2(image2)}
+                    'dense_features2': self.feature_extraction_image2(image2, live)}
         if not torch.is_grad_enabled() and image1.is_cuda and image1.dtype == torch.float32:
             from c2m_amd import ops as _ops
-            return _ops.f16_range_guard(self, both, image1.device)
+
+            def fused():
+                return both(_ops.ref_live_extent_shared(image2) if self.ref_band else None)
+            return _ops.f16_range_guard(self, fused, image1.device)
         return both()
diff --git a/c2-matching_amd/mmsr/models/archs/corres_generation_arch.py b/c2-matching_amd/mmsr/models/archs/corres_generation_arch.py
--- a/c2-matching_amd/mmsr/models/archs/corres_generation_arch.py
+++ b/c2-matching_amd/mmsr/models/archs/corres_generation_arch.py
@@ -64,6 +64,7 @@
         self.vgg = VGGFeatureExtractor(layer_name_list=vgg_layer_list, vgg_type=vgg_type)
         self.vgg.grouped8_taps = ('relu1_1',)
         self.vgg.fast_conv = True
+        self.vgg.ref_band = True
 
     def index_to_flow(self, max_idx):
         h, w = max_idx.shape
diff --git a/c2-matching_amd/mmsr/models/archs/vgg_arch.py b/c2-matching_amd/mmsr/models/archs/vgg_arch.py
--- a/c2-matching_amd/mmsr/models/archs/vgg_arch.py
+++ b/c2-matching_amd/mmsr/models/archs/vgg_arch.py
@@ -124,7 +124,8 @@
             return _ops.f16_range_guard(self, lambda: _ops.vgg_stack_forward(
                 self.vgg_net._modules, x, taps=self.layer_name_list, mean=self.mean if self.use_input_norm else None,
                 std=self.std if self.use_input_norm else None, grouped8_taps=getattr(self, 'grouped8_taps', ()),
-                fast=getattr(self, 'fast_conv', False)), x.device)
+                fast=getattr(self, 'fast_conv', False),
+                live=_ops.ref_live_extent_shared(x) if getattr(self, 'ref_band', False) else None), x.device)
         if self.use_input_norm:
             x = (x - self.mean) / self.std
         taps = {}
diff --git a/c2-matching_amd/mmsr/models/ref_restoration_model.py b/c2-matching_amd/mmsr/models/ref_restoration_model.py
--- a/c2-matching_amd/mmsr/models/ref_restoration_model.py
+++ b/c2-matching_amd/mmsr/models/ref_restoration_model.py
@@ -229,6 +229,9 @@
         self.net_g.eval()
         with torch.no_grad():
             def whole():
+                if self.img_ref.is_cuda:
+                    from c2m_amd import ops as _ops
+                    _ops.ref_live_extent_shared(self.img_ref)
                 self._correspondence()
                 return self.net_g(self.img_in_lq, self.pre_offset, self.img_ref_feat)
             if self.img_in_lq.is_cuda:
diff --git a/include/c2m_hip.h b/include/c2m_hip.h
--- a/include/c2m_hip.h
+++ b/include/c2m_hip.h
@@ -157,6 +157,8 @@
 int c2m_conv3x3_relayout_split_f32(c2m_stream_t stream, const float* weight, int Cin, int Cout, int pieces, void* wr);
 int c2m_conv3x3_relayout_split_multi(c2m_stream_t stream, const long long* jobs, int njobs, long long nblocks, int any_f16);
 int c2m_conv3x3_nhwc_f32(c2m_stream_t stream, const c2m_conv3x3_desc* desc);
+int c2m_conv3x3_nhwc_roi_f32(c2m_stream_t stream, const c2m_conv3x3_desc* desc, int roi_tiles_y, int roi_tiles_x);
+int c2m_conv3x3_roi_tile(int rgb64, int* tile_h, int* tile_w);
 
 int c2m_conv3x3_relayout_split_dgrad_f32(c2m_stream_t stream, const float* weight , int Cin, int Cout,
                                          int pieces, void* wr);
@@ -169,6 +171,15 @@
                           const float* bias, const float* mean, const float* std_, int act, float slope, float* out,
                           int out_pix_pitch, int out_row_pitch, long long out_img_pitch, float* out2, int out2_row_pitch,
                           long long out2_plane_pitch, long long out2_img_pitch);
+int c2m_conv3x3_rgb64_roi_f32(c2m_stream_t stream, const float* image, int B, int H, int W, const float* weight,
+                              const float* bias, const float* mean, const float* std_, int act, float slope, float* out,
+                              int out_pix_pitch, int out_row_pitch, long long out_img_pitch, float* out2, int out2_row_pitch,
+                              long long out2_plane_pitch, long long out2_img_pitch, int roi_tiles_y, int roi_tiles_x);
+
+int c2m_ref_live_extent_f32(c2m_stream_t stream, const float* image, int B, int H, int W, int* extent);
+int c2m_band_fill_f32(c2m_stream_t stream, float* dst, int B, int C, int H, int W, int cpg, int d_pix_pitch, int d_row_pitch,
+                      long long d_plane_pitch, long long d_img_pitch, const float* tmpl, int Ht, int Wt, int t_pix_pitch,
+                      int t_row_pitch, long long t_plane_pitch, int roi_h, int roi_w, int margin_y, int margin_x, int planar);
 
 int c2m_index_to_flow_f32(c2m_stream_t stream, const int64_t* max_idx, int B, int hq, int wq, float* flow);
 
```

Result: faster. 118.2, median of 6 (+1.2%).
